# sml2004/CUDA-powered-mesh-handling-and-Iterative-solvers

Measured on NVIDIA B200. Metric: cg_iters_per_s, higher is better.
Workload: dtype f64

## Files before the change

cuda-powered-mesh-handling-and-iterative-solvers_b200/csrc/krylov.cu:

```cuda
#include <cstdlib>

#include "spmv_dev.cuh"

namespace femb {

struct CGState {
  double rs_old, rs_new, pAp, alpha, beta;
  int it, stop, status, iterations;
  unsigned int ticket1, ticket2;
  int fin, fin_status;
};

template <int THREADS>
__device__ __forceinline__ void cg_k1_epilogue_n(double dot, double* __restrict__ partial, CGState* __restrict__ st, double eps, int guards) {
  const double t = block_sum<THREADS>(dot);
  __shared__ bool last;
  if (threadIdx.x == 0) {
    partial[blockIdx.x] = t;
    __threadfence();
    last = atomicAdd(&st->ticket1, 1u) == gridDim.x - 1;
  }
  __syncthreads();
  if (last) {
    __threadfence();
    double a = 0.0;
    for (int k = threadIdx.x; k < (int)gridDim.x; k += THREADS) a += ((volatile double*)partial)[k];
    a = block_sum<THREADS>(a);
    if (threadIdx.x == 0) {
      st->ticket1 = 0;
      st->pAp = a;
      if (guards && (fabs(a) < eps || a < 0.0)) {
        st->stop = 1, st->status = 1, st->iterations = st->it + 1;
      } else {
        const double alpha = st->rs_old / (a + eps);
        st->alpha = alpha;
        if (guards && !isfinite(alpha)) st->stop = 1, st->status = 1, st->iterations = st->it + 1;
      }
    }
  }
}

__device__ __forceinline__ void cg_k1_epilogue(double dot, double* __restrict__ partial, CGState* __restrict__ st, double eps, int guards) {
  cg_k1_epilogue_n<SPMV_THREADS>(dot, partial, st, eps, guards);
}

template <int THREADS>
__device__ __forceinline__ void cg_k1_epilogue3_n(double dot, double e0, double e1, double* __restrict__ partial, CGState* __restrict__ st,
                                                  double eps, int guards, double tol) {
  const double t0 = block_sum<THREADS>(dot), t1 = block_sum<THREADS>(e0), t2 = block_sum<THREADS>(e1);
  const int G = gridDim.x;
  __shared__ bool last;
  if (threadIdx.x == 0) {
    partial[blockIdx.x] = t0, partial[G + blockIdx.x] = t1, partial[2 * G + blockIdx.x] = t2;
    __threadfence();
    last = atomicAdd(&st->ticket1, 1u) == gridDim.x - 1;
  }
  __syncthreads();
  if (last) {
    __threadfence();
    double a = 0.0, b = 0.0, c = 0.0;
    for (int k = threadIdx.x; k < G; k += THREADS)
      a += ((volatile double*)partial)[k], b += ((volatile double*)partial)[G + k], c += ((volatile double*)partial)[2 * G + k];
    a = block_sum<THREADS>(a), b = block_sum<THREADS>(b), c = block_sum<THREADS>(c);
    if (threadIdx.x == 0) {
      st->ticket1 = 0;
      st->pAp = a;
      const double rs = st->rs_old, alpha = rs / (a + eps);
      if (guards && (fabs(a) < eps || a < 0.0 || !isfinite(alpha))) {
        st->stop = 1, st->status = 1, st->iterations = st->it + 1;
      } else {
        double rs_new = rs - 2.0 * alpha * b + alpha * alpha * c;
        if (!(rs_new > 0.0)) rs_new = 0.0;
        const double beta = rs_new / (rs + eps);
        st->alpha = alpha, st->beta = beta, st->rs_new = rs_new;
        st->fin = 0;
        if (guards && !isfinite(beta)) st->fin = 1, st->fin_status = 1;
      }
    }
  }
}

template <int L, bool FUSED>
__global__ void __launch_bounds__(SPMV_THREADS) spmv_kernel(long long n, const int* __restrict__ crow, const int* __restrict__ col,
                                                            const double* __restrict__ val, const double* __restrict__ x,
                                                            double* __restrict__ y, const unsigned char* __restrict__ mask,
                                                            double* __restrict__ partial, CGState* __restrict__ st, double eps, int guards,
                                                            const double* __restrict__ rvec, double tol, const double* __restrict__ wvec) {
  if (st && st->stop) return;
  const bool accumulate = (guards & 2) != 0;
  guards &= 1;
  double e0 = 0.0, e1 = 0.0;
  const int sub = threadIdx.x % L;
  const long long group = (blockIdx.x * (long long)blockDim.x + threadIdx.x) / L;
  const long long ngroups = ((long long)gridDim.x * blockDim.x) / L;
  double dot = 0.0;
  for (long long r0 = 0; r0 < n; r0 += ngroups) {
    const long long r = r0 + group;
    double sum = 0.0;
    if (r < n) {
      const int s = __ldg(crow + r), e = __ldg(crow + r + 1);
      int j = s + sub;
      for (; j + L < e; j += 2 * L) {
        const int c0 = ld_stream(col + j), c1 = ld_stream(col + j + L);
        const double v0 = ld_stream(val + j), v1 = ld_stream(val + j + L);
        sum += v0 * __ldg(x + c0);
        sum += v1 * __ldg(x + c1);
      }
      if (j < e) sum += ld_stream(val + j) * __ldg(x + ld_stream(col + j));
    }
#pragma unroll
    for (int o = L / 2; o > 0; o >>= 1) sum += __shfl_xor_sync(0xffffffffu, sum, o);
    if (r < n && sub == 0) {
      if (accumulate) sum += y[r];
      if (FUSED) {
        if (mask && !mask[r]) sum = 0.0;
        dot += sum * __ldg(x + r);
        if (rvec) {
          const double w = wvec ? wvec[r] : 1.0;
          e0 += sum * (w * rvec[r]), e1 += sum * (sum * w);
        }
      }
      y[r] = sum;
    }
  }
  if (FUSED) {
    if (rvec) cg_k1_epilogue3_n<SPMV_THREADS>(dot, e0, e1, partial, st, eps, guards, tol);
    else cg_k1_epilogue(dot, partial, st, eps, guards);
  }
}

template <int LR, bool FUSED>
__global__ void __launch_bounds__(SPMV_THREADS) spmv_stream_kernel(long long n, const int* __restrict__ crow, const int* __restrict__ col,
                                                                   const double* __restrict__ val, const double* __restrict__ x,
                                                                   double* __restrict__ y, const unsigned char* __restrict__ mask,
                                                                   double* __restrict__ partial, CGState* __restrict__ st, double eps,
                                                                   int guards, const double* __restrict__ rvec, double tol,
                                                                   const double* __restrict__ wvec) {
  if (st && st->stop) return;
  const double dot = spmv_stream_rows<LR, true>(n, crow, col, val, x, y, mask, (guards & 2) != 0, FUSED);
  if (FUSED) cg_k1_epilogue(dot, partial, st, eps, guards & 1);
}

template <int LR, bool FUSED>
__global__ void __launch_bounds__(TMA_THREADS) spmv_tma_kernel(long long n, long long nnz, const int* __restrict__ crow, const int* __restrict__ col,
                                                               const double* __restrict__ val, const double* __restrict__ x,
                                                               double* __restrict__ y, const unsigned char* __restrict__ mask,
                                                               double* __restrict__ partial, CGState* __restrict__ st, double eps, int guards,
                                                               const double* __restrict__ rvec, double tol, long long pin,
                                                               const double* __restrict__ wvec) {
  pdl_launch_dependents();
  double extra[2] = {0.0, 0.0};
  const double dot = spmv_tma_rows<LR, true, TMA_THREADS, TMA_STAGES, TMA_CAP, NoHaloWait, PdlWait>(
      n, nnz, crow, col, val, x, y, mask, (guards & 2) != 0, FUSED, 0x7fffffffffffffffll, NoHaloWait(), rvec, rvec ? extra : nullptr, PdlWait(),
      st ? &st->stop : nullptr, pin, wvec);
  if (st && st->stop) return;
  if (FUSED) {
    if (rvec) cg_k1_epilogue3_n<TMA_THREADS>(dot, extra[0], extra[1], partial, st, eps, guards & 1, tol);
    else cg_k1_epilogue_n<TMA_THREADS>(dot, partial, st, eps, guards & 1);
  }
}

template <bool FUSED>
__global__ void __launch_bounds__(TMA_THREADS) spmv_tma16_kernel(long long n, long long nnz, const int* __restrict__ crow, const int* __restrict__ col,
                                                                 const double* __restrict__ val, const double* __restrict__ x,
                                                                 double* __restrict__ y, const unsigned char* __restrict__ mask,
                                                                 double* __restrict__ partial, CGState* __restrict__ st, double eps, int guards,
                                                                 const double* __restrict__ rvec, double tol, long long pin,
                                                                 const double* __restrict__ wvec, const unsigned short* __restrict__ col16,
                                                                 const unsigned char* __restrict__ tile_ok) {
  pdl_launch_dependents();
  double extra[2] = {0.0, 0.0};
  const double dot = spmv_tma16_rows<TMA16_STAGES, TMA16_CAP>(n, nnz, crow, col, col16, tile_ok, val, x, y, mask, (guards & 2) != 0, FUSED, rvec,
                                                             rvec ? extra : nullptr, st ? &st->stop : nullptr, pin, wvec);
  if (st && st->stop) return;
  if (FUSED) {
    if (rvec) cg_k1_epilogue3_n<TMA_THREADS>(dot, extra[0], extra[1], partial, st, eps, guards & 1, tol);
    else cg_k1_epilogue_n<TMA_THREADS>(dot, partial, st, eps, guards & 1);
  }
}

__global__ void __launch_bounds__(TMA_THREADS) idx16_encode_kernel(long long n, const int* __restrict__ crow, const int* __restrict__ col,
                                                                   unsigned short* __restrict__ col16, unsigned char* __restrict__ tile_ok,
                                                                   int* __restrict__ bad) {
  const long long ntiles = (n + TMA_THREADS - 1) / TMA_THREADS;
  for (long long t = blockIdx.x; t < ntiles; t += gridDim.x) {
    const long long r = t * TMA_THREADS + threadIdx.x;
    bool ok = true;
    if (r < n) {
      const int a = __ldg(crow + r), b = __ldg(crow + r + 1);
      long long prev = r;
      for (int j = a; j < b; ++j) {
        const long long c = __ldg(col + j), d = j == a ? prev - c : c - prev;
        ok = ok && d >= (j == a ? 0 : 1) && d <= 65535;
        col16[j] = (unsigned short)d;
        prev = c;
      }
    }
    ok = __syncthreads_and(ok);
    if (threadIdx.x == 0) {
      tile_ok[t] = ok ? 1 : 0;
      if (!ok) atomicAdd(bad, 1);
    }
  }
}

template <int LR, bool FUSED>
__global__ void __launch_bounds__(TMA_THREADS) spmv_bsr3_tma_kernel(long long nb, long long nnzb, const int* __restrict__ brow,
                                                                    const int* __restrict__ bcol, const double* __restrict__ bval,
                                                                    const double* __restrict__ x, double* __restrict__ y,
                                                                    const unsigned char* __restrict__ mask, double* __restrict__ partial,
                                                                    CGState* __restrict__ st, double eps, int guards,
                                                                    const double* __restrict__ rvec, double tol, const double* __restrict__ wvec) {
  if (st && st->stop) return;
  const double dot = spmv_bsr3_tma_rows<LR, true>(nb, nnzb, brow, bcol, bval, x, y, mask, (guards & 2) != 0, FUSED);
  if (FUSED) cg_k1_epilogue_n<TMA_THREADS>(dot, partial, st, eps, guards & 1);
}

constexpr int BSRV_THREADS = 256;
template <bool FUSED, int U, bool MERGED>
__global__ void __launch_bounds__(BSRV_THREADS) spmv_bsr3_vec_kernel(long long nb, long long nnzb, const int* __restrict__ brow,
                                                                     const int* __restrict__ bcol, const double* __restrict__ bval,
                                                                     const double* __restrict__ x, double* __restrict__ y,
                                                                     const unsigned char* __restrict__ mask, double* __restrict__ partial,
                                                                     CGState* __restrict__ st, double eps, int guards,
                                                                     const double* __restrict__ rvec, double tol, const double* __restrict__ wvec) {
  if (st && st->stop) return;
  const bool accumulate = (guards & 2) != 0;
  guards &= 1;
  double e0 = 0.0, e1 = 0.0;
  const int lane = threadIdx.x & 31;
  const int boff = lane / 9, pos = lane - 9 * boff, cx = pos % 3;
  const bool active = lane < 27;
  const long long gw = (blockIdx.x * (long long)blockDim.x + threadIdx.x) >> 5, nw = ((long long)gridDim.x * blockDim.x) >> 5;
  double dot = 0.0;
  const bool owner = lane == 0 || lane == 3 || lane == 6;
  for (long long r = gw; r < nb; r += nw) {
    const int a = __ldg(brow + r), e = __ldg(brow + r + 1);
    double r_own = 0.0, w_own = 1.0;
    if (MERGED && owner) {
      r_own = rvec[3 * r + lane / 3];
      if (wvec) w_own = wvec[3 * r + lane / 3];
    }
    double acc = 0.0;
    if (active) {
      int b = a + boff;
      for (; b + 3 * (U - 1) < e; b += 3 * U) {
        double v[U], xv[U];
#pragma unroll
        for (int q = 0; q < U; ++q) {
          v[q] = ld_stream(bval + (size_t)(b + 3 * q) * 9 + pos);
          xv[q] = __ldg(x + 3ll * ld_stream(bcol + b + 3 * q) + cx);
        }
#pragma unroll
        for (int q = 0; q < U; ++q) acc += v[q] * xv[q];
      }
      for (; b < e; b += 3) acc += ld_stream(bval + (size_t)b * 9 + pos) * __ldg(x + 3ll * ld_stream(bcol + b) + cx);
    }
    acc += __shfl_down_sync(0xffffffffu, acc, 9) + __shfl_down_sync(0xffffffffu, acc, 18);
    acc += __shfl_down_sync(0xffffffffu, acc, 1) + __shfl_down_sync(0xffffffffu, acc, 2);
    if (lane == 0 || lane == 3 || lane == 6) {
      const long long i = 3 * r + lane / 3;
      double sv = acc;
      if (accumulate) sv += y[i];
      if (FUSED) {
        if (mask && !mask[i]) sv = 0.0;
        dot += sv * __ldg(x + i);
        if (MERGED) e0 += sv * (w_own * r_own), e1 += sv * (sv * w_own);
      }
      y[i] = sv;
    }
  }
  if (FUSED) {
    if (MERGED) cg_k1_epilogue3_n<BSRV_THREADS>(dot, e0, e1, partial, st, eps, guards, tol);
    else cg_k1_epilogue_n<BSRV_THREADS>(dot, partial, st, eps, guards);
  }
}

template <bool TO_BSR>
__global__ void csr_bsr3_permute_kernel(long long nb, const int* __restrict__ brow, const double* __restrict__ in, double* __restrict__ out) {
  const int lane = threadIdx.x & 31;
  const long long w0 = (blockIdx.x * (long long)blockDim.x + threadIdx.x) >> 5, nw = ((long long)gridDim.x * blockDim.x) >> 5;
  for (long long i = w0; i < nb; i += nw) {
    const long long a = brow[i];
    const int len = brow[i + 1] - (int)a, row = 3 * len;
    for (int t = lane; t < 9 * len; t += 32) {
      const int al = t / row, rem = t - al * row, slot = rem / 3, be = rem - 3 * slot;
      const long long ci = 9 * a + t, bi = 9 * (a + slot) + 3 * al + be;
      if (TO_BSR) out[bi] = in[ci];
      else out[ci] = in[bi];
    }
  }
}

__global__ void bsr3_jacobi_kernel(long long nb, const int* __restrict__ brow, const int* __restrict__ bcol, const double* __restrict__ bval,
                                   const unsigned char* __restrict__ mask, double* __restrict__ minv) {
  for (long long r = blockIdx.x * (long long)blockDim.x + threadIdx.x; r < nb; r += (long long)gridDim.x * blockDim.x) {
    int lo = brow[r], hi = brow[r + 1];
    const int end = hi;
    while (lo < hi) {
      const int mid = (lo + hi) >> 1;
      if (bcol[mid] < r) lo = mid + 1;
      else hi = mid;
    }
    const bool found = lo < end && bcol[lo] == r;
    for (int i = 0; i < 3; ++i) {
      const double d = found ? bval[(size_t)lo * 9 + 4 * i] : 0.0;
      minv[3 * r + i] = (d != 0.0 && (!mask || mask[3 * r + i])) ? 1.0 / d : 0.0;
    }
  }
}

constexpr int VEC_THREADS = 256;

__global__ void __launch_bounds__(VEC_THREADS) cg_update_kernel(long long n, double* __restrict__ u, double* __restrict__ r,
                                                                const double* __restrict__ p, const double* __restrict__ Ap,
                                                                const double* __restrict__ minv, double* __restrict__ partial,
                                                                CGState* __restrict__ st, double tol, double eps, int guards, int max_iter) {
  if (st->stop) return;
  const double alpha = st->alpha;
  double dot = 0.0;
  for (long long i = blockIdx.x * (long long)blockDim.x + threadIdx.x; i < n; i += (long long)gridDim.x * blockDim.x) {
    const double pi = p[i], ri = r[i] - alpha * Ap[i];
    u[i] += alpha * pi;
    r[i] = ri;
    dot += minv ? ri * (minv[i] * ri) : ri * ri;
  }
  const double t = block_sum<VEC_THREADS>(dot);
  __shared__ bool last;
  if (threadIdx.x == 0) {
    partial[blockIdx.x] = t;
    __threadfence();
    last = atomicAdd(&st->ticket2, 1u) == gridDim.x - 1;
  }
  __syncthreads();
  if (last) {
    __threadfence();
    double a = 0.0;
    for (int k = threadIdx.x; k < (int)gridDim.x; k += VEC_THREADS) a += ((volatile double*)partial)[k];
    a = block_sum<VEC_THREADS>(a);
    if (threadIdx.x == 0) {
      st->ticket2 = 0;
      st->rs_new = a;
      if (sqrt(a) < tol) {
        st->stop = 1, st->status = 0, st->iterations = st->it + 1;
      } else {
        const double beta = a / (st->rs_old + eps);
        st->beta = beta;
        if (guards && !isfinite(beta)) {
          st->stop = 1, st->status = 1, st->iterations = st->it + 1;
        } else {
          st->rs_old = a;
          st->it += 1;
          if (st->it >= max_iter) st->stop = 2, st->status = 2, st->iterations = max_iter;
        }
      }
    }
  }
}

__global__ void __launch_bounds__(VEC_THREADS) cg_direction_kernel(long long n, const double* __restrict__ r, double* __restrict__ p,
                                                                   const double* __restrict__ minv, const CGState* __restrict__ st) {
  if (st->stop == 1) return;
  const double beta = st->beta;
  for (long long i = blockIdx.x * (long long)blockDim.x + threadIdx.x; i < n; i += (long long)gridDim.x * blockDim.x) {
    const double z = minv ? minv[i] * r[i] : r[i];
    p[i] = z + beta * p[i];
  }
}

__global__ void __launch_bounds__(VEC_THREADS) cg_merged_kernel(long long n, double* __restrict__ u, double* __restrict__ r, double* __restrict__ p,
                                                                const double* __restrict__ Ap, const double* __restrict__ minv,
                                                                double* __restrict__ partial, CGState* __restrict__ st, int max_iter, double tol) {
  pdl_launch_dependents();
  pdl_wait();
  if (st->stop) return;
  const double alpha = st->alpha, beta = st->beta;
  const bool move_p = st->fin == 0;
  double dot = 0.0;
  for (long long i = blockIdx.x * (long long)blockDim.x + threadIdx.x; i < n; i += (long long)gridDim.x * blockDim.x) {
    const double pi = p[i], ri = r[i] - alpha * Ap[i];
    const double zi = minv ? minv[i] * ri : ri;
    u[i] += alpha * pi;
    r[i] = ri;
    dot += ri * zi;
    if (move_p) p[i] = zi + beta * pi;
  }
  const double t = block_sum<VEC_THREADS>(dot);
  __shared__ bool last;
  if (threadIdx.x == 0) {
    partial[blockIdx.x] = t;
    __threadfence();
    last = atomicAdd(&st->ticket2, 1u) == gridDim.x - 1;
  }
  __syncthreads();
  if (last) {
    __threadfence();
    double a = 0.0;
    for (int k = threadIdx.x; k < (int)gridDim.x; k += VEC_THREADS) a += ((volatile double*)partial)[k];
    a = block_sum<VEC_THREADS>(a);
    if (threadIdx.x == 0) {
      st->ticket2 = 0;
      st->rs_new = a;
      if (sqrt(a) < tol) {
        st->stop = 1, st->status = 0, st->iterations = st->it + 1;
      } else if (!move_p) {
        st->stop = 1, st->status = st->fin_status, st->iterations = st->it + 1;
      } else {
        st->rs_old = a;
        st->it += 1;
        if (st->it >= max_iter) st->stop = 2, st->status = 2, st->iterations = max_iter;
      }
    }
  }
}

__global__ void cg_mask_kernel(long long n, double* __restrict__ u, const unsigned char* __restrict__ mask) {
  for (long long i = blockIdx.x * (long long)blockDim.x + threadIdx.x; i < n; i += (long long)gridDim.x * blockDim.x)
    if (!mask[i]) u[i] = 0.0;
}

__global__ void __launch_bounds__(VEC_THREADS) cg_init_kernel(long long n, const double* __restrict__ F, const double* __restrict__ Au,
                                                              const unsigned char* __restrict__ mask, const double* __restrict__ minv,
                                                              double* __restrict__ r, double* __restrict__ p, double* __restrict__ partial) {
  double dot = 0.0;
  for (long long i = blockIdx.x * (long long)blockDim.x + threadIdx.x; i < n; i += (long long)gridDim.x * blockDim.x) {
    double ri = F[i] - Au[i];
    if (mask && !mask[i]) ri = 0.0;
    const double z = minv ? minv[i] * ri : ri;
    r[i] = ri;
    p[i] = z;
    dot += ri * z;
  }
  const double t = block_sum<VEC_THREADS>(dot);
  if (threadIdx.x == 0) partial[blockIdx.x] = t;
}

__global__ void __launch_bounds__(VEC_THREADS) cg_init_finish(int nparts, const double* __restrict__ partial, CGState* __restrict__ st,
                                                              int max_iter) {
  double a = 0.0;
  for (int k = threadIdx.x; k < nparts; k += VEC_THREADS) a += partial[k];
  a = block_sum<VEC_THREADS>(a);
  if (threadIdx.x == 0) {
    CGState s;
    memset(&s, 0, sizeof(s));
    s.rs_old = a;
    s.rs_new = a;
    if (max_iter <= 0) s.stop = 2, s.status = 2;
    *st = s;
  }
}

__global__ void jacobi_kernel(long long n, const int* __restrict__ crow, const int* __restrict__ col, const double* __restrict__ val,
                              const unsigned char* __restrict__ mask, double* __restrict__ minv) {
  for (long long r = blockIdx.x * (long long)blockDim.x + threadIdx.x; r < n; r += (long long)gridDim.x * blockDim.x) {
    double d = 0.0;
    int lo = crow[r], hi = crow[r + 1];
    while (lo < hi) {
      const int mid = (lo + hi) >> 1;
      if (col[mid] < r) lo = mid + 1;
      else hi = mid;
    }
    if (lo < crow[r + 1] && col[lo] == r) d = val[lo];
    minv[r] = (d != 0.0 && (!mask || mask[r])) ? 1.0 / d : 0.0;
  }
}

static int pick_lanes(long long n, long long nnz, int block = 1) {
  static const bool bsr_tma = getenv("FEMB_BSR_TMA") != nullptr;
  static const int bsrv_unroll = getenv("FEMB_BSRV_UNROLL") ? atoi(getenv("FEMB_BSRV_UNROLL")) : 4;
  if (block == 3) return bsr_tma ? 200 + bsr_pick_lr(n / 3, nnz) : (bsrv_unroll == 2 ? 301 : 300);
  const double avg = n > 0 ? (double)nnz / (double)n : 1.0;
  static const bool force_vector = getenv("FEMB_SPMV_VECTOR") != nullptr, force_stream = getenv("FEMB_SPMV_STREAM") != nullptr;
  if (force_vector) return -(avg <= 3 ? 2 : avg <= 6 ? 4 : avg <= 24 ? 8 : avg <= 48 ? 16 : 32);
  static const bool force_tma = getenv("FEMB_SPMV_TMA") != nullptr;
  if (!force_stream && !force_tma && avg >= 64.0) return -32;
  if (!force_stream) return 100 + tma_pick_lr(n, nnz);
  for (int lr = 1; lr <= 32; lr *= 2)
    if ((SPMV_THREADS / lr) * avg * 1.25 <= STREAM_CAP) return lr;
  return 32;
}

static thread_local long long nnz_hint = 0;
static thread_local bool pdl_hint = false;
static thread_local long long pin_hint = 0;
static thread_local const unsigned short* col16_hint = nullptr;
static thread_local const unsigned char* tile_ok_hint = nullptr;

template <bool FUSED>
static void launch_spmv(int lanes, int grid, cudaStream_t s, long long n, const int* crow, const int* col, const double* val, const double* x,
                        double* y, const unsigned char* mask, double* partial, CGState* st, double eps, int guards,
                        const double* rvec = nullptr, double tol = 0.0, const double* wvec = nullptr) {
#define FEMB_SPMV_ARGS n, crow, col, val, x, y, mask, partial, st, eps, guards, rvec, tol, wvec
#define FEMB_TMA(LRV)                                                                                                              \
  {                                                                                                                                \
    cudaFuncSetAttribute(spmv_tma_kernel<LRV, FUSED>, cudaFuncAttributeMaxDynamicSharedMemorySize, (int)TMA_SMEM);                 \
    launch_pdl(spmv_tma_kernel<LRV, FUSED>, grid, TMA_THREADS, TMA_SMEM, s, pdl_hint, n, nnz_hint, crow, col, val, x, y, mask, partial, st, eps, \
               guards, rvec, tol, pin_hint, wvec);                                                                               \
  }
#define FEMB_BSR(LRV)                                                                                                              \
  {                                                                                                                                \
    cudaFuncSetAttribute(spmv_bsr3_tma_kernel<LRV, FUSED>, cudaFuncAttributeMaxDynamicSharedMemorySize, (int)BSR_SMEM);            \
    spmv_bsr3_tma_kernel<LRV, FUSED><<<grid, TMA_THREADS, BSR_SMEM, s>>>(n / 3, nnz_hint, crow, col, val, x, y, mask, partial, st, eps, guards, rvec, tol, wvec); \
  }
  switch (lanes) {
#define FEMB_BSRV(UV)                                                                                                              \
  {                                                                                                                                \
    if (FUSED && rvec)                                                                                                             \
      spmv_bsr3_vec_kernel<FUSED, UV, FUSED><<<grid, BSRV_THREADS, 0, s>>>(n / 3, nnz_hint, crow, col, val, x, y, mask, partial, st, eps, guards, rvec, tol, wvec); \
    else                                                                                                                           \
      spmv_bsr3_vec_kernel<FUSED, UV, false><<<grid, BSRV_THREADS, 0, s>>>(n / 3, nnz_hint, crow, col, val, x, y, mask, partial, st, eps, guards, rvec, tol, wvec); \
  }
    case 300: FEMB_BSRV(4) break;
    case 301: FEMB_BSRV(2) break;
    case 201: FEMB_BSR(1) break;
    case 202: FEMB_BSR(2) break;
    case 204: FEMB_BSR(4) break;
    case 208: FEMB_BSR(8) break;
    case 216: FEMB_BSR(16) break;
    case 232: FEMB_BSR(32) break;
    case 101:
      if (col16_hint) {
        cudaFuncSetAttribute(spmv_tma16_kernel<FUSED>, cudaFuncAttributeMaxDynamicSharedMemorySize, (int)TMA16_SMEM);
        launch_pdl(spmv_tma16_kernel<FUSED>, grid, TMA_THREADS, TMA16_SMEM, s, pdl_hint, n, nnz_hint, crow, col, val, x, y, mask, partial, st,
                   eps, guards, rvec, tol, pin_hint, wvec, col16_hint, tile_ok_hint);
      } else {
        FEMB_TMA(1)
      }
      break;
    case 102: FEMB_TMA(2) break;
    case 104: FEMB_TMA(4) break;
    case 108: FEMB_TMA(8) break;
    case 116: FEMB_TMA(16) break;
    case 132: FEMB_TMA(32) break;
    case 1: spmv_stream_kernel<1, FUSED><<<grid, SPMV_THREADS, 0, s>>>(FEMB_SPMV_ARGS); break;
    case 2: spmv_stream_kernel<2, FUSED><<<grid, SPMV_THREADS, 0, s>>>(FEMB_SPMV_ARGS); break;
    case 4: spmv_stream_kernel<4, FUSED><<<grid, SPMV_THREADS, 0, s>>>(FEMB_SPMV_ARGS); break;
    case 8: spmv_stream_kernel<8, FUSED><<<grid, SPMV_THREADS, 0, s>>>(FEMB_SPMV_ARGS); break;
    case 16: spmv_stream_kernel<16, FUSED><<<grid, SPMV_THREADS, 0, s>>>(FEMB_SPMV_ARGS); break;
    case 32: spmv_stream_kernel<32, FUSED><<<grid, SPMV_THREADS, 0, s>>>(FEMB_SPMV_ARGS); break;
    case -2: spmv_kernel<2, FUSED><<<grid, SPMV_THREADS, 0, s>>>(FEMB_SPMV_ARGS); break;
    case -4: spmv_kernel<4, FUSED><<<grid, SPMV_THREADS, 0, s>>>(FEMB_SPMV_ARGS); break;
    case -8: spmv_kernel<8, FUSED><<<grid, SPMV_THREADS, 0, s>>>(FEMB_SPMV_ARGS); break;
    case -16: spmv_kernel<16, FUSED><<<grid, SPMV_THREADS, 0, s>>>(FEMB_SPMV_ARGS); break;
    default: spmv_kernel<32, FUSED><<<grid, SPMV_THREADS, 0, s>>>(FEMB_SPMV_ARGS); break;
  }
#undef FEMB_TMA
#undef FEMB_BSR
#undef FEMB_BSRV
#undef FEMB_SPMV_ARGS
}

static int spmv_grid(long long n, int lanes, bool merged = false) {
  if (lanes == 300 || lanes == 301) {
    static int fit[2][2] = {{0, 0}, {0, 0}};
    if (!fit[0][0]) {
      cudaOccupancyMaxActiveBlocksPerMultiprocessor(&fit[0][0], spmv_bsr3_vec_kernel<true, 4, false>, BSRV_THREADS, 0);
      cudaOccupancyMaxActiveBlocksPerMultiprocessor(&fit[1][0], spmv_bsr3_vec_kernel<true, 2, false>, BSRV_THREADS, 0);
      cudaOccupancyMaxActiveBlocksPerMultiprocessor(&fit[0][1], spmv_bsr3_vec_kernel<true, 4, true>, BSRV_THREADS, 0);
      cudaOccupancyMaxActiveBlocksPerMultiprocessor(&fit[1][1], spmv_bsr3_vec_kernel<true, 2, true>, BSRV_THREADS, 0);
      for (auto& f : fit)
        for (int& v : f)
          if (v < 1) v = 1;
    }
    const int per_sm = getenv("FEMB_BSRV_CTAS") ? atoi(getenv("FEMB_BSRV_CTAS")) : fit[lanes - 300][merged ? 1 : 0];
    const long long ctas = (n / 3 + BSRV_THREADS / 32 - 1) / (BSRV_THREADS / 32);
    return (int)std::max<long long>(1, std::min<long long>(ctas, (long long)SMS * per_sm));
  }
  if (lanes >= 200) return tma_grid(n / 3, lanes - 200);
  if (lanes >= 100) return tma_grid(n, lanes - 100);
  const long long rows_per_block = SPMV_THREADS / (lanes < 0 ? -lanes : lanes);
  const long long tiles = std::max<long long>(1, (n + rows_per_block - 1) / rows_per_block);
  if (lanes < 0) return (int)std::min<long long>(tiles, (long long)SMS * 8);
  const long long max_ctas = SMS * 32;
  const long long per = (tiles + max_ctas - 1) / max_ctas;
  return (int)((tiles + per - 1) / per);
}

}

using namespace femb;

extern "C" int femb_spmv(int64_t n, int64_t nnz, const int32_t* crow, const int32_t* col, const double* val, const double* x, double* y,
                         femb_stream stream) {
  FEMB_CHECK_ARG(n >= 0, "n >= 0");
  if (n == 0) return FEMB_OK;
  cudaStream_t s = as_stream(stream);
  spmv_apply_env_once();
  const int lanes = pick_lanes(n, nnz);
  nnz_hint = nnz;
  launch_spmv<false>(lanes, spmv_grid(n, lanes), s, n, crow, col, val, x, y, nullptr, nullptr, nullptr, 0.0, 0);
  FEMB_LAUNCH_CHECK();
  return FEMB_OK;
}

extern "C" int femb_csr_jacobi(int64_t n, const int32_t* crow, const int32_t* col, const double* val, const uint8_t* mask, double* minv,
                               femb_stream stream) {
  if (n == 0) return FEMB_OK;
  jacobi_kernel<<<grid_for(n, 256), 256, 0, as_stream(stream)>>>(n, crow, col, val, mask, minv);
  FEMB_LAUNCH_CHECK();
  return FEMB_OK;
}

struct CsrRef {
  long long nnz;
  const int *crow, *col;
  const double* val;
  int block = 1;
};

static int cg_solve_impl(int64_t n, int nmat, const CsrRef* mats, const double* F, const uint8_t* mask, const double* minv, double* u,
                         double* work, double tol, int max_iter, double eps, int check_every, femb_cg_result* result_host,
                         femb_stream stream) {
  FEMB_CHECK_ARG(n > 0 && nmat >= 1 && nmat <= 8 && F && u && work && result_host, "null pointer / n <= 0 / nmat not in 1..8");
  if (check_every < 1) check_every = 16;
  spmv_apply_env_once();
  SolveCtx* ctx = solve_ctx(as_stream(stream));
  if (!ctx) return FEMB_ERR_CUDA;
  cudaStream_t s = ctx->stream;
  const int guards = minv ? 0 : 1;
  if (minv) eps = 0.0;
  double *r = work, *p = work + n, *Ap = work + 2 * n;
  int lanes[8], g1[8], gmax = 1;
  for (int m = 0; m < nmat; ++m) lanes[m] = pick_lanes(n, mats[m].nnz, mats[m].block);
  static const bool classic_env = getenv("FEMB_CG_CLASSIC") != nullptr;
  const int ll = lanes[nmat - 1];
  static const bool bsr_merged = getenv("FEMB_BSR_MERGED") != nullptr;
  const bool merged = !classic_env && ((ll >= 300 && bsr_merged) || (ll >= 100 && ll < 200) || ll < 0);
  static const bool idx32_env = getenv("FEMB_SPMV_IDX32") != nullptr;
  bool use16 = !idx32_env && merged && nmat == 1 && lanes[0] == 101 && max_iter >= 16;
  const long long ntiles16 = (n + TMA_THREADS - 1) / TMA_THREADS;
  const size_t flags_off = 256, col16_off = flags_off + (((size_t)ntiles16 + 255) & ~(size_t)255);
  if (use16) {
    const size_t need16 = col16_off + 2 * (((size_t)mats[0].nnz + 7) & ~(size_t)7);
    if (ctx->idx16_bytes < need16) {
      if (ctx->graph_exec) cudaGraphExecDestroy(ctx->graph_exec), ctx->graph_exec = nullptr, ctx->graph_key_bytes = 0;
      FEMB_CUDA(cudaStreamSynchronize(s));
      if (ctx->idx16) cudaFree(ctx->idx16);
      ctx->idx16 = nullptr, ctx->idx16_bytes = 0;
      if (cudaMalloc(&ctx->idx16, need16) == cudaSuccess) ctx->idx16_bytes = need16;
      else ctx->idx16 = nullptr, use16 = false, cudaGetLastError();
    }
  }
  if (use16) {
    unsigned char* base16 = static_cast<unsigned char*>(ctx->idx16);
    static_assert(2 * sizeof(CGState) + sizeof(int) <= 512 && 512 + sizeof(int) <= SOLVE_PINNED_BYTES, "pinned status buffer");
    int* bad_host = reinterpret_cast<int*>(static_cast<unsigned char*>(ctx->pinned) + 512);
    FEMB_CUDA(cudaMemsetAsync(base16, 0, sizeof(int), s));
    idx16_encode_kernel<<<(int)std::min<long long>(ntiles16, (long long)SMS * 16), TMA_THREADS, 0, s>>>(
        n, mats[0].crow, mats[0].col, reinterpret_cast<unsigned short*>(base16 + col16_off), base16 + flags_off, reinterpret_cast<int*>(base16));
    FEMB_LAUNCH_CHECK();
    FEMB_CUDA(cudaMemcpyAsync(bad_host, base16, sizeof(int), cudaMemcpyDeviceToHost, s));
    FEMB_CUDA(cudaStreamSynchronize(s));
    use16 = (long long)*bad_host * 100 <= ntiles16;
  }
  const unsigned short* col16 = use16 ? reinterpret_cast<const unsigned short*>(static_cast<unsigned char*>(ctx->idx16) + col16_off) : nullptr;
  const unsigned char* tile_ok = use16 ? static_cast<unsigned char*>(ctx->idx16) + flags_off : nullptr;
  for (int m = 0; m < nmat; ++m) {
    g1[m] = spmv_grid(n, lanes[m], merged && m == nmat - 1);
    if (use16) g1[m] = tma16_grid(n);
    gmax = std::max(gmax, g1[m]);
  }
  const int g2 = grid_for(n, VEC_THREADS, 8);
  static const int vec_waves = getenv("FEMB_VEC_WAVES") ? atoi(getenv("FEMB_VEC_WAVES")) : 8;
  const int g2v = grid_for(n, VEC_THREADS, vec_waves);
  const size_t need = 256 + sizeof(double) * (size_t)std::max(3 * gmax, g2);
  if (ctx->dev_scratch_bytes < need) {
    if (ctx->graph_exec) cudaGraphExecDestroy(ctx->graph_exec), ctx->graph_exec = nullptr, ctx->graph_key_bytes = 0;
    FEMB_CUDA(cudaStreamSynchronize(s));
    if (ctx->dev_scratch) cudaFree(ctx->dev_scratch);
    ctx->dev_scratch = nullptr, ctx->dev_scratch_bytes = 0;
    FEMB_CUDA(cudaMalloc(&ctx->dev_scratch, need + need / 2));
    ctx->dev_scratch_bytes = need + need / 2;
  }
  static_assert(sizeof(CGState) <= 256, "state slot");
  CGState* st = static_cast<CGState*>(ctx->dev_scratch);
  double* partial = reinterpret_cast<double*>(static_cast<unsigned char*>(ctx->dev_scratch) + 256);
  if (mask) cg_mask_kernel<<<g2, VEC_THREADS, 0, s>>>(n, u, mask);
  col16_hint = col16, tile_ok_hint = tile_ok;
  for (int m = 0; m < nmat; ++m)
    nnz_hint = mats[m].nnz, launch_spmv<false>(lanes[m], g1[m], s, n, mats[m].crow, mats[m].col, mats[m].val, u, Ap, nullptr, nullptr, nullptr, 0.0, m ? 2 : 0);
  col16_hint = nullptr, tile_ok_hint = nullptr;
  cg_init_kernel<<<g2, VEC_THREADS, 0, s>>>(n, F, Ap, mask, minv, r, p, partial);
  cg_init_finish<<<1, VEC_THREADS, 0, s>>>(g2, partial, st, max_iter);
  FEMB_LAUNCH_CHECK();
  struct GraphKey {
    long long n;
    int nmat, check_every, max_iter, guards, merged, pdl, lanes[8], g1[8], g2, g2v;
    long long nnz[8];
    const void *crow[8], *col[8], *val[8];
    int block[8];
    const void *mask, *minv, *u, *work, *st, *partial;
    double tol, eps;
    long long pin;
    const void* col16;
  } key;
  memset(&key, 0, sizeof(key));
  static_assert(sizeof(GraphKey) <= sizeof(ctx->graph_key), "graph key buffer");
  key.n = n, key.nmat = nmat, key.check_every = check_every, key.max_iter = max_iter, key.guards = guards, key.merged = merged ? 1 : 0;
  key.pdl = pdl_mode(), key.g2 = g2, key.g2v = g2v, key.mask = mask, key.minv = minv, key.u = u, key.work = work, key.st = st, key.partial = partial;
  key.tol = tol, key.eps = eps, key.pin = spmv_pin_entries(mats[nmat - 1].nnz), key.col16 = col16;
  for (int m = 0; m < nmat; ++m) {
    key.lanes[m] = lanes[m], key.g1[m] = g1[m];
    key.nnz[m] = mats[m].nnz, key.crow[m] = mats[m].crow, key.col[m] = mats[m].col, key.val[m] = mats[m].val, key.block[m] = mats[m].block;
  }
  static const bool no_cache = getenv("FEMB_NO_GRAPH_CACHE") != nullptr;
  cudaGraph_t graph = nullptr;
  cudaGraphExec_t exec = nullptr;
  if (!no_cache && ctx->graph_exec && ctx->graph_key_bytes == sizeof(key) && memcmp(ctx->graph_key, &key, sizeof(key)) == 0) exec = ctx->graph_exec;
  if (!exec) {
  FEMB_CUDA(cudaStreamBeginCapture(s, cudaStreamCaptureModeThreadLocal));
  for (int k = 0; k < check_every; ++k) {
    for (int m = 0; m + 1 < nmat; ++m)
      nnz_hint = mats[m].nnz, launch_spmv<false>(lanes[m], g1[m], s, n, mats[m].crow, mats[m].col, mats[m].val, p, Ap, nullptr, nullptr, st, 0.0, m ? 2 : 0);
    const int last = nmat - 1;
    nnz_hint = mats[last].nnz;
    if (merged) {
      const bool pdl = pdl_enabled() && nmat == 1 && lanes[last] >= 100 && lanes[last] < 200;
      pdl_hint = pdl && k > 0 && (pdl_mode() & 2);
      pin_hint = pdl ? spmv_pin_entries(mats[last].nnz) : 0;
      col16_hint = col16, tile_ok_hint = tile_ok;
      launch_spmv<true>(lanes[last], g1[last], s, n, mats[last].crow, mats[last].col, mats[last].val, p, Ap, mask, partial, st, eps,
                        guards | (last ? 2 : 0), r, tol, minv);
      pdl_hint = false, pin_hint = 0, col16_hint = nullptr, tile_ok_hint = nullptr;
      launch_pdl(cg_merged_kernel, g2v, VEC_THREADS, 0, s, pdl && (pdl_mode() & 1), n, u, r, p, Ap, minv, partial, st, max_iter, tol);
    } else {
      launch_spmv<true>(lanes[last], g1[last], s, n, mats[last].crow, mats[last].col, mats[last].val, p, Ap, mask, partial, st, eps,
                        guards | (last ? 2 : 0));
      cg_update_kernel<<<g2, VEC_THREADS, 0, s>>>(n, u, r, p, Ap, minv, partial, st, tol, eps, guards, max_iter);
      cg_direction_kernel<<<g2, VEC_THREADS, 0, s>>>(n, r, p, minv, st);
    }
  }
  cudaError_t ce = cudaStreamEndCapture(s, &graph);
  if (ce != cudaSuccess) {
    set_error(std::string("cudaStreamEndCapture: ") + cudaGetErrorString(ce));
    return FEMB_ERR_CUDA;
  }
  FEMB_CUDA(cudaGraphInstantiate(&exec, graph, 0));
  cudaGraphDestroy(graph);
  FEMB_CUDA(cudaGraphUpload(exec, s));
  if (ctx->graph_exec) cudaGraphExecDestroy(ctx->graph_exec);
  ctx->graph_exec = exec, ctx->graph_key_bytes = sizeof(key);
  memcpy(ctx->graph_key, &key, sizeof(key));
  }
  static_assert(2 * sizeof(CGState) <= SOLVE_PINNED_BYTES, "pinned status buffer");
  CGState* hst = static_cast<CGState*>(ctx->pinned);
  cudaEvent_t* ev = ctx->poll_ev;
  cudaEvent_t* tev = ctx->time_ev;
  int rc = FEMB_OK;
  const int launches = (max_iter + check_every - 1) / check_every;
  hst[0].stop = hst[1].stop = 0;
  bool stopped = false;
  cudaEventRecord(tev[0], s);
  for (int l = 0; l < launches && !stopped; ++l) {
    if (cudaGraphLaunch(exec, s) != cudaSuccess || cudaMemcpyAsync(&hst[l & 1], st, sizeof(CGState), cudaMemcpyDeviceToHost, s) != cudaSuccess ||
        cudaEventRecord(ev[l & 1], s) != cudaSuccess) {
      set_error(std::string("CG graph launch: ") + cudaGetErrorString(cudaGetLastError()));
      rc = FEMB_ERR_CUDA;
      break;
    }
    if (l >= 1) {
      cudaEventSynchronize(ev[(l - 1) & 1]);
      stopped = hst[(l - 1) & 1].stop != 0;
    }
  }
  cudaEventRecord(tev[1], s);
  CGState* fin = &hst[0];
  if (rc == FEMB_OK) {
    if (cudaMemcpyAsync(fin, st, sizeof(CGState), cudaMemcpyDeviceToHost, s) != cudaSuccess || cudaStreamSynchronize(s) != cudaSuccess) {
      set_error(std::string("CG final state: ") + cudaGetErrorString(cudaGetLastError()));
      rc = FEMB_ERR_CUDA;
    }
  }
  float ms = 0.f;
  if (rc == FEMB_OK) cudaEventElapsedTime(&ms, tev[0], tev[1]);
  if (rc != FEMB_OK) {
    cudaGraphExecDestroy(ctx->graph_exec);
    ctx->graph_exec = nullptr, ctx->graph_key_bytes = 0;
    return rc;
  }
  result_host->iterations = fin->stop ? fin->iterations : max_iter;
  result_host->status = fin->stop ? fin->status : 2;
  result_host->rs = fin->rs_new;
  result_host->loop_ms = ms;
  result_host->index_bytes = use16 ? 2 : 4;
  return FEMB_OK;
}

extern "C" int femb_cg_solve(int64_t n, int64_t nnz, const int32_t* crow, const int32_t* col, const double* val, const double* F,
                             const uint8_t* mask, const double* minv, double* u, double* work, double tol, int max_iter, double eps,
                             int check_every, femb_cg_result* result_host, femb_stream stream) {
  FEMB_CHECK_ARG(crow && col && val, "null CSR pointer");
  const CsrRef m{nnz, crow, col, val, 1};
  return cg_solve_impl(n, 1, &m, F, mask, minv, u, work, tol, max_iter, eps, check_every, result_host, stream);
}

extern "C" int femb_spmv_bsr3(int64_t nb, int64_t nnzb, const int32_t* brow, const int32_t* bcol, const double* bval, const double* x,
                              double* y, femb_stream stream) {
  FEMB_CHECK_ARG(nb >= 0 && nnzb >= 0, "nb >= 0, nnzb >= 0");
  if (nb == 0) return FEMB_OK;
  cudaStream_t s = as_stream(stream);
  const int lanes = pick_lanes(3 * nb, nnzb, 3);
  nnz_hint = nnzb;
  launch_spmv<false>(lanes, spmv_grid(3 * nb, lanes), s, 3 * nb, brow, bcol, bval, x, y, nullptr, nullptr, nullptr, 0.0, 0);
  FEMB_LAUNCH_CHECK();
  return FEMB_OK;
}

extern "C" int femb_cg_solve_bsr3(int64_t nb, int64_t nnzb, const int32_t* brow, const int32_t* bcol, const double* bval, const double* F,
                                  const uint8_t* mask, const double* minv, double* u, double* work, double tol, int max_iter, double eps,
                                  int check_every, femb_cg_result* result_host, femb_stream stream) {
  FEMB_CHECK_ARG(brow && bcol && bval, "null BSR pointer");
  const CsrRef m{nnzb, brow, bcol, bval, 3};
  return cg_solve_impl(3 * nb, 1, &m, F, mask, minv, u, work, tol, max_iter, eps, check_every, result_host, stream);
}

extern "C" int femb_csr_bsr3_convert(int to_bsr, int64_t nb, const int32_t* brow, const double* in, double* out, femb_stream stream) {
  FEMB_CHECK_ARG(nb >= 0 && brow && in && out && in != out, "nb >= 0, non-null distinct buffers");
  if (nb == 0) return FEMB_OK;
  const int grid = grid_for(nb * 32, 256, 32);
  if (to_bsr) csr_bsr3_permute_kernel<true><<<grid, 256, 0, as_stream(stream)>>>(nb, brow, in, out);
  else csr_bsr3_permute_kernel<false><<<grid, 256, 0, as_stream(stream)>>>(nb, brow, in, out);
  FEMB_LAUNCH_CHECK();
  return FEMB_OK;
}

extern "C" int femb_bsr3_jacobi(int64_t nb, const int32_t* brow, const int32_t* bcol, const double* bval, const uint8_t* mask, double* minv,
                                femb_stream stream) {
  if (nb == 0) return FEMB_OK;
  bsr3_jacobi_kernel<<<grid_for(nb, 256), 256, 0, as_stream(stream)>>>(nb, brow, bcol, bval, mask, minv);
  FEMB_LAUNCH_CHECK();
  return FEMB_OK;
}

extern "C" int femb_cg_solve_multi(int64_t n, int nmat, const int64_t* nnz_host, const int32_t* const* crow_host,
                                   const int32_t* const* col_host, const double* const* val_host, const double* F, const uint8_t* mask,
                                   const double* minv, double* u, double* work, double tol, int max_iter, double eps, int check_every,
                                   femb_cg_result* result_host, femb_stream stream) {
  FEMB_CHECK_ARG(nmat >= 1 && nmat <= 8 && nnz_host && crow_host && col_host && val_host, "nmat in 1..8, non-null arrays");
  CsrRef m[8];
  for (int k = 0; k < nmat; ++k) m[k] = CsrRef{nnz_host[k], crow_host[k], col_host[k], val_host[k], 1};
  return cg_solve_impl(n, nmat, m, F, mask, minv, u, work, tol, max_iter, eps, check_every, result_host, stream);
}

namespace femb {

__global__ void __launch_bounds__(VEC_THREADS) cg_dot_kernel(long long n, const double* __restrict__ p, const double* __restrict__ Ap,
                                                             double* __restrict__ partial, CGState* __restrict__ st) {
  if (st->stop) return;
  double dot = 0.0;
  for (long long i = blockIdx.x * (long long)blockDim.x + threadIdx.x; i < n; i += (long long)gridDim.x * blockDim.x) dot += p[i] * Ap[i];
  cg_k1_epilogue_n<VEC_THREADS>(dot, partial, st, 0.0, 0);
}

}

extern "C" int femb_cg_solve_operator(int64_t n, femb_apply_fn apply, void* ctx, const double* R, double* u, double* work, double tol,
                                      int max_iter, int check_every, femb_cg_result* result_host, femb_stream stream) {
  FEMB_CHECK_ARG(n > 0 && apply && R && u && work && result_host, "null pointer / n <= 0");
  if (check_every < 1) check_every = 8;
  cudaStream_t s = as_stream(stream);
  double *r = work, *p = work + n, *Ap = work + 2 * n;
  const int g2 = grid_for(n, VEC_THREADS, 8);
  Scratch scr(s);
  double* partial;
  CGState* st;
  FEMB_CUDA(scr.alloc(&partial, (size_t)g2));
  FEMB_CUDA(scr.alloc(&st, 1));
  cudaEvent_t t0, t1;
  FEMB_CUDA(cudaEventCreate(&t0));
  FEMB_CUDA(cudaEventCreate(&t1));
  int rc = FEMB_OK;
  CGState h;
  memset(&h, 0, sizeof(h));
  auto fail = [&](const char* what) {
    set_error(what);
    rc = FEMB_ERR_ARG;
  };
  if (apply(ctx, u, Ap, stream) != 0) fail("femb_cg_solve_operator: the operator callback failed");
  if (rc == FEMB_OK) {
    cg_init_kernel<<<g2, VEC_THREADS, 0, s>>>(n, R, Ap, nullptr, nullptr, r, p, partial);
    cg_init_finish<<<1, VEC_THREADS, 0, s>>>(g2, partial, st, max_iter);
    cudaEventRecord(t0, s);
    for (int it = 0; it < max_iter && rc == FEMB_OK; ++it) {
      if (apply(ctx, p, Ap, stream) != 0) {
        fail("femb_cg_solve_operator: the operator callback failed");
        break;
      }
      cg_dot_kernel<<<g2, VEC_THREADS, 0, s>>>(n, p, Ap, partial, st);
      cg_update_kernel<<<g2, VEC_THREADS, 0, s>>>(n, u, r, p, Ap, nullptr, partial, st, tol, 0.0, 0, max_iter);
      cg_direction_kernel<<<g2, VEC_THREADS, 0, s>>>(n, r, p, nullptr, st);
      if ((it + 1) % check_every == 0 || it + 1 == max_iter) {
        if (cudaMemcpyAsync(&h, st, sizeof(CGState), cudaMemcpyDeviceToHost, s) != cudaSuccess || cudaStreamSynchronize(s) != cudaSuccess) {
          set_error(std::string("femb_cg_solve_operator: ") + cudaGetErrorString(cudaGetLastError()));
          rc = FEMB_ERR_CUDA;
          break;
        }
        if (h.stop) break;
      }
    }
    cudaEventRecord(t1, s);
  }
  if (rc == FEMB_OK) {
    if (cudaMemcpyAsync(&h, st, sizeof(CGState), cudaMemcpyDeviceToHost, s) != cudaSuccess || cudaStreamSynchronize(s) != cudaSuccess) {
      set_error(std::string("femb_cg_solve_operator: ") + cudaGetErrorString(cudaGetLastError()));
      rc = FEMB_ERR_CUDA;
    }
  }
  float ms = 0.f;
  if (rc == FEMB_OK) cudaEventElapsedTime(&ms, t0, t1);
  cudaEventDestroy(t0);
  cudaEventDestroy(t1);
  if (rc != FEMB_OK) {
    cudaStreamSynchronize(s);
    return rc;
  }
  result_host->iterations = h.stop ? h.iterations : max_iter;
  result_host->status = h.stop ? h.status : 2;
  result_host->rs = h.rs_new;
  result_host->loop_ms = ms;
  result_host->index_bytes = 0;
  return FEMB_OK;
}
```

cuda-powered-mesh-handling-and-iterative-solvers_b200/csrc/spmv_dev.cuh:

```cuda
#pragma once
#include <cstdlib>

#include "common.cuh"

namespace femb {

constexpr int SPMV_THREADS = 256;
constexpr int STREAM_CAP = 5632;

__device__ __forceinline__ double ld_stream(const double* p) {
  double v;
  asm volatile("ld.global.nc.L1::no_allocate.f64 %0, [%1];" : "=d"(v) : "l"(p));
  return v;
}
__device__ __forceinline__ int ld_stream(const int* p) {
  int v;
  asm volatile("ld.global.nc.L1::no_allocate.s32 %0, [%1];" : "=r"(v) : "l"(p));
  return v;
}
template <bool NC>
__device__ __forceinline__ double ld_x(const double* p) {
  if (NC) return __ldg(p);
  return *p;
}

struct NoHaloWait {
  __device__ __forceinline__ void operator()() const {}
};

template <int LR, bool NC, typename Wait = NoHaloWait>
__device__ __forceinline__ double spmv_stream_rows(long long n, const int* __restrict__ crow, const int* __restrict__ col,
                                                   const double* __restrict__ val, const double* __restrict__ x, double* __restrict__ y,
                                                   const unsigned char* __restrict__ mask, bool accumulate, bool fused,
                                                   long long halo_row = 0x7fffffffffffffffll, Wait wait = Wait()) {
  constexpr int R = SPMV_THREADS / LR;
  __shared__ double prod[STREAM_CAP];
  __shared__ int rp[R + 1];
  const int tid = threadIdx.x, sub = tid % LR, lr = tid / LR;
  double dot = 0.0;
  bool waited = false;
  for (long long r0 = (long long)blockIdx.x * R; r0 < n; r0 += (long long)gridDim.x * R) {
    const int nr = (int)min((long long)R, n - r0);
    if (!waited && r0 + nr > halo_row) {
      wait();
      waited = true;
    }
    double x_own = 0.0, y_prev = 0.0;
    bool keep = true;
    if (lr < nr && sub == 0) {
      if (fused) {
        x_own = ld_x<NC>(x + r0 + lr);
        if (mask) keep = mask[r0 + lr] != 0;
      }
      if (accumulate) y_prev = y[r0 + lr];
    }
    for (int t = tid; t <= nr; t += SPMV_THREADS) rp[t] = __ldg(crow + r0 + t);
    __syncthreads();
    const int s = rp[0], e = rp[nr];
    const bool fits = (e - s) <= STREAM_CAP;
    if (fits) {
      int j = s + tid;
      for (; j + 3 * SPMV_THREADS < e; j += 4 * SPMV_THREADS) {
        int c[4];
        double v[4];
#pragma unroll
        for (int q = 0; q < 4; ++q) c[q] = ld_stream(col + j + q * SPMV_THREADS), v[q] = ld_stream(val + j + q * SPMV_THREADS);
#pragma unroll
        for (int q = 0; q < 4; ++q) prod[j - s + q * SPMV_THREADS] = v[q] * ld_x<NC>(x + c[q]);
      }
      for (; j < e; j += SPMV_THREADS) prod[j - s] = ld_stream(val + j) * ld_x<NC>(x + ld_stream(col + j));
    }
    __syncthreads();
    double sum = 0.0;
    if (lr < nr) {
      const int a = rp[lr], b = rp[lr + 1];
      if (fits) {
        for (int j = a - s + sub; j < b - s; j += LR) sum += prod[j];
      } else {
        for (int j = a + sub; j < b; j += LR) sum += ld_stream(val + j) * ld_x<NC>(x + ld_stream(col + j));
      }
    }
#pragma unroll
    for (int o = LR / 2; o > 0; o >>= 1) sum += __shfl_xor_sync(0xffffffffu, sum, o);
    if (lr < nr && sub == 0) {
      const long long r = r0 + lr;
      if (accumulate) sum += y_prev;
      if (fused) {
        if (!keep) sum = 0.0;
        dot += sum * x_own;
      }
      y[r] = sum;
    }
    __syncthreads();
  }
  return dot;
}

__device__ __forceinline__ unsigned smem_u32(const void* p) { return static_cast<unsigned>(__cvta_generic_to_shared(p)); }
__device__ __forceinline__ void mbar_init(unsigned long long* bar, unsigned count) {
  asm volatile("mbarrier.init.shared::cta.b64 [%0], %1;" ::"r"(smem_u32(bar)), "r"(count));
}
__device__ __forceinline__ void mbar_expect_tx(unsigned long long* bar, unsigned bytes) {
  asm volatile("mbarrier.arrive.expect_tx.shared::cta.b64 _, [%0], %1;" ::"r"(smem_u32(bar)), "r"(bytes) : "memory");
}
__device__ __forceinline__ void mbar_wait(unsigned long long* bar, unsigned parity) {
  asm volatile(
      "{\n\t.reg .pred p;\n\t"
      "WAIT_LOOP:\n\t"
      "mbarrier.try_wait.parity.shared::cta.b64 p, [%0], %1;\n\t"
      "@p bra WAIT_DONE;\n\t"
      "bra WAIT_LOOP;\n\t"
      "WAIT_DONE:\n\t}" ::"r"(smem_u32(bar)),
      "r"(parity)
      : "memory");
}
__device__ __forceinline__ void bulk_g2s(void* dst, const void* src, unsigned bytes, unsigned long long* bar) {
  asm volatile("cp.async.bulk.shared::cluster.global.mbarrier::complete_tx::bytes [%0], [%1], %2, [%3];" ::"r"(smem_u32(dst)), "l"(src),
               "r"(bytes), "r"(smem_u32(bar))
               : "memory");
}

__device__ __forceinline__ unsigned long long l2_evict_first_policy() {
  unsigned long long pol;
  asm volatile("createpolicy.fractional.L2::evict_first.b64 %0, 1.0;" : "=l"(pol));
  return pol;
}
__device__ __forceinline__ void bulk_g2s_hint(void* dst, const void* src, unsigned bytes, unsigned long long* bar, unsigned long long pol) {
  asm volatile("cp.async.bulk.shared::cluster.global.mbarrier::complete_tx::bytes.L2::cache_hint [%0], [%1], %2, [%3], %4;" ::"r"(smem_u32(dst)),
               "l"(src), "r"(bytes), "r"(smem_u32(bar)), "l"(pol)
               : "memory");
}
__device__ __forceinline__ unsigned long long l2_evict_last_policy() {
  unsigned long long pol;
  asm volatile("createpolicy.fractional.L2::evict_last.b64 %0, 1.0;" : "=l"(pol));
  return pol;
}
static __device__ int g_spmv_l2_hint = 1;
static inline void spmv_apply_env_once() {
  static thread_local int done_for = -1;
  int dev = 0;
  if (cudaGetDevice(&dev) != cudaSuccess || dev == done_for) return;
  done_for = dev;
  if (const char* e = getenv("FEMB_SPMV_L2HINT")) {
    const int v = atoi(e);
    cudaMemcpyToSymbol(g_spmv_l2_hint, &v, sizeof(int));
  }
}
inline long long spmv_pin_entries(long long nnz) {
  static const double env_mb = getenv("FEMB_SPMV_PIN_MB") ? atof(getenv("FEMB_SPMV_PIN_MB")) : -1.0;
  const double bytes = 12.0 * (double)nnz;
  double pin_mb = env_mb;
  if (pin_mb < 0.0) pin_mb = 0.0;
  return (long long)std::min(bytes, pin_mb * 1e6) / 12;
}

__device__ __forceinline__ void pdl_launch_dependents() { asm volatile("griddepcontrol.launch_dependents;" ::: "memory"); }
__device__ __forceinline__ void pdl_wait() { asm volatile("griddepcontrol.wait;" ::: "memory"); }
struct PdlWait {
  __device__ __forceinline__ void operator()() const { pdl_wait(); }
};
struct NoDep {
  __device__ __forceinline__ void operator()() const {}
};

template <typename... KArgs, typename... Args>
inline cudaError_t launch_pdl(void (*kern)(KArgs...), int grid, int block, size_t smem, cudaStream_t s, bool pdl, Args... args) {
  cudaLaunchConfig_t cfg = {};
  cfg.gridDim = dim3((unsigned)grid), cfg.blockDim = dim3((unsigned)block), cfg.dynamicSmemBytes = smem, cfg.stream = s;
  cudaLaunchAttribute at[1];
  at[0].id = cudaLaunchAttributeProgrammaticStreamSerialization;
  at[0].val.programmaticStreamSerializationAllowed = 1;
  cfg.attrs = at, cfg.numAttrs = pdl ? 1 : 0;
  return cudaLaunchKernelEx(&cfg, kern, static_cast<KArgs>(args)...);
}
inline int pdl_mode() {
  static const int m = getenv("FEMB_NO_PDL") ? 0 : (getenv("FEMB_PDL_MODE") ? atoi(getenv("FEMB_PDL_MODE")) : 2);
  return m;
}
inline bool pdl_enabled() { return pdl_mode() != 0; }

constexpr int TMA_THREADS = 128, TMA_STAGES = 2, TMA_CAP = 2304, TMA_CTAS_PER_SM = 4;
constexpr size_t TMA_SMEM = (size_t)TMA_STAGES * TMA_CAP * 12;

template <int LR, bool NC, int THREADS = TMA_THREADS, int STAGES = TMA_STAGES, int CAP = TMA_CAP, typename Wait = NoHaloWait,
          typename Dep = NoDep>
__device__ __forceinline__ double spmv_tma_rows(long long n, long long nnz, const int* __restrict__ crow, const int* __restrict__ col,
                                                const double* __restrict__ val, const double* __restrict__ x, double* __restrict__ y,
                                                const unsigned char* __restrict__ mask, bool accumulate, bool fused,
                                                long long halo_row = 0x7fffffffffffffffll, Wait wait = Wait(),
                                                const double* __restrict__ rvec = nullptr, double* extra = nullptr, Dep dep = Dep(),
                                                const int* stop = nullptr, long long pin = 0, const double* __restrict__ wvec = nullptr) {
  constexpr int R = THREADS / LR;
  extern __shared__ __align__(128) unsigned char tma_smem[];
  double* vbuf = reinterpret_cast<double*>(tma_smem);
  int* cbuf = reinterpret_cast<int*>(tma_smem + sizeof(double) * STAGES * CAP);
  __shared__ unsigned long long full[STAGES];
  __shared__ int base[STAGES];
  const int tid = threadIdx.x, sub = tid % LR, lr = tid / LR;
  const long long ntiles = (n + R - 1) / R;
  const bool use_hint = g_spmv_l2_hint != 0;
  const unsigned long long pol = l2_evict_first_policy(), pol_keep = l2_evict_last_policy();
  if (tid == 0) {
    for (int s = 0; s < STAGES; ++s) mbar_init(&full[s], 1);
    asm volatile("fence.mbarrier_init.release.cluster;" ::: "memory");
  }
  __syncthreads();
  auto bounds = [&](long long k, int& a, int& b) {
    const long long t = blockIdx.x + k * gridDim.x;
    a = b = 0;
    if (t < ntiles) a = __ldg(crow + t * R), b = __ldg(crow + min(n, t * R + R));
  };
  auto stage_tile = [&](long long k, int a, int b) {
    if (blockIdx.x + k * gridDim.x >= ntiles) return;
    const int s = (int)(k % STAGES);
    const int a0 = a & ~3, cnt = (b - a0 + 3) & ~3;
    if (cnt > CAP || (long long)a0 + cnt > nnz || cnt == 0) {
      base[s] = -1;
      return;
    }
    base[s] = a0;
    asm volatile("fence.proxy.async.shared::cta;" ::: "memory");
    mbar_expect_tx(&full[s], (unsigned)cnt * 12u);
    if (use_hint) {
      const unsigned long long pl = (long long)a0 + cnt <= pin ? pol_keep : pol;
      bulk_g2s_hint(vbuf + (size_t)s * CAP, val + a0, (unsigned)cnt * 8u, &full[s], pl);
      bulk_g2s_hint(cbuf + (size_t)s * CAP, col + a0, (unsigned)cnt * 4u, &full[s], pl);
    } else {
      bulk_g2s(vbuf + (size_t)s * CAP, val + a0, (unsigned)cnt * 8u, &full[s]);
      bulk_g2s(cbuf + (size_t)s * CAP, col + a0, (unsigned)cnt * 4u, &full[s]);
    }
  };
  int na = 0, nb = 0;
  if (tid == 0) {
    for (int k = 0; k < STAGES - 1; ++k) {
      bounds(k, na, nb);
      stage_tile(k, na, nb);
    }
    bounds(STAGES - 1, na, nb);
  }
  double dot = 0.0;
  unsigned phase_bits = 0;
  bool waited = false;
  dep();
  if (stop) {
    __shared__ int stop_sh;
    if (tid == 0) stop_sh = *(volatile const int*)stop;
    __syncthreads();
    if (stop_sh) {
      for (int k = 0; k < STAGES - 1; ++k)
        if (blockIdx.x + (long long)k * gridDim.x < ntiles && base[k % STAGES] >= 0) mbar_wait(&full[k % STAGES], 0u);
      return 0.0;
    }
  }
  for (long long k = 0;; ++k) {
    const long long t = blockIdx.x + k * gridDim.x;
    if (t >= ntiles) break;
    const int s = (int)(k % STAGES);
    if (!waited && min(n, t * R + R) > halo_row) {
      wait();
      waited = true;
    }
    if (tid == 0) {
      stage_tile(k + STAGES - 1, na, nb);
      bounds(k + STAGES, na, nb);
    }
    const long long r = t * R + lr;
    int ra = 0, rb = 0;
    double x_own = 0.0, y_prev = 0.0, r_own = 0.0, w_own = 1.0;
    bool keep = true;
    if (r < n) {
      ra = __ldg(crow + r), rb = __ldg(crow + r + 1);
      if (sub == 0) {
        if (fused) {
          x_own = ld_x<NC>(x + r);
          if (mask) keep = mask[r] != 0;
          if (rvec) r_own = rvec[r];
          if (wvec) w_own = wvec[r];
        }
        if (accumulate) y_prev = y[r];
      }
    }
    __syncthreads();
    const int a0 = base[s];
    double sum = 0.0;
    if (a0 >= 0) {
      mbar_wait(&full[s], (phase_bits >> s) & 1u);
      phase_bits ^= 1u << s;
      const double* vs = vbuf + (size_t)s * CAP - a0;
      const int* cs = cbuf + (size_t)s * CAP - a0;
      int j = ra + sub;
      for (; j + 7 * LR < rb; j += 8 * LR) {
        double xv[8];
#pragma unroll
        for (int q = 0; q < 8; ++q) xv[q] = ld_x<NC>(x + cs[j + q * LR]);
#pragma unroll
        for (int q = 0; q < 8; ++q) sum += vs[j + q * LR] * xv[q];
      }
      {
        double xv[7];
#pragma unroll
        for (int q = 0; q < 7; ++q) xv[q] = (j + q * LR < rb) ? ld_x<NC>(x + cs[j + q * LR]) : 0.0;
#pragma unroll
        for (int q = 0; q < 7; ++q)
          if (j + q * LR < rb) sum += vs[j + q * LR] * xv[q];
      }
    } else {
      for (int j = ra + sub; j < rb; j += LR) sum += ld_stream(val + j) * ld_x<NC>(x + ld_stream(col + j));
    }
#pragma unroll
    for (int o = LR / 2; o > 0; o >>= 1) sum += __shfl_xor_sync(0xffffffffu, sum, o);
    if (r < n && sub == 0) {
      if (accumulate) sum += y_prev;
      if (fused) {
        if (!keep) sum = 0.0;
        dot += sum * x_own;
        if (extra) extra[0] += sum * (w_own * r_own), extra[1] += sum * (sum * w_own);
      }
      y[r] = sum;
    }
    __syncthreads();
  }
  return dot;
}

inline int tma_pick_lr(long long n, long long nnz) {
  const double avg = n > 0 ? (double)nnz / (double)n : 1.0;
  for (int lr = 1; lr <= 32; lr *= 2)
    if ((TMA_THREADS / lr) * avg * 1.15 <= TMA_CAP) return lr;
  return 32;
}
inline int tma_grid(long long n, int lr) {
  const long long tiles = (n + TMA_THREADS / lr - 1) / (TMA_THREADS / lr);
  return (int)std::max<long long>(1, std::min<long long>(tiles, (long long)SMS * TMA_CTAS_PER_SM));
}

#ifndef FEMB_TMA16_STAGES
#define FEMB_TMA16_STAGES 2
#endif
#ifndef FEMB_TMA16_CAP
#define FEMB_TMA16_CAP 2176
#endif
#ifndef FEMB_TMA16_CTAS
#define FEMB_TMA16_CTAS 5
#endif
constexpr int TMA16_STAGES = FEMB_TMA16_STAGES, TMA16_CAP = FEMB_TMA16_CAP, TMA16_CTAS_PER_SM = FEMB_TMA16_CTAS;
constexpr size_t TMA16_SMEM = (size_t)TMA16_STAGES * TMA16_CAP * 10;
inline int tma16_grid(long long n) {
  const long long tiles = (n + TMA_THREADS - 1) / TMA_THREADS;
  return (int)std::max<long long>(1, std::min<long long>(tiles, (long long)SMS * TMA16_CTAS_PER_SM));
}

template <int STAGES, int CAP>
__device__ __forceinline__ double spmv_tma16_rows(long long n, long long nnz, const int* __restrict__ crow, const int* __restrict__ col,
                                                  const unsigned short* __restrict__ col16, const unsigned char* __restrict__ tile_ok,
                                                  const double* __restrict__ val, const double* __restrict__ x, double* __restrict__ y,
                                                  const unsigned char* __restrict__ mask, bool accumulate, bool fused,
                                                  const double* __restrict__ rvec, double* extra, const int* stop, long long pin,
                                                  const double* __restrict__ wvec) {
  static_assert(CAP % 8 == 0, "16-byte aligned stages");
  constexpr int R = TMA_THREADS;
  extern __shared__ __align__(128) unsigned char tma_smem[];
  double* vbuf = reinterpret_cast<double*>(tma_smem);
  unsigned short* dbuf = reinterpret_cast<unsigned short*>(tma_smem + sizeof(double) * STAGES * CAP);
  __shared__ unsigned long long full[STAGES];
  __shared__ int base[STAGES];
  const int tid = threadIdx.x;
  const long long ntiles = (n + R - 1) / R;
  const bool use_hint = g_spmv_l2_hint != 0;
  const unsigned long long pol = l2_evict_first_policy(), pol_keep = l2_evict_last_policy();
  if (tid == 0) {
    for (int s = 0; s < STAGES; ++s) mbar_init(&full[s], 1);
    asm volatile("fence.mbarrier_init.release.cluster;" ::: "memory");
  }
  __syncthreads();
  auto bounds = [&](long long k, int& a, int& b, int& ok) {
    const long long t = blockIdx.x + k * gridDim.x;
    a = b = ok = 0;
    if (t < ntiles) a = __ldg(crow + t * R), b = __ldg(crow + min(n, t * R + R)), ok = __ldg(tile_ok + t);
  };
  auto stage_tile = [&](long long k, int a, int b, int ok) {
    if (blockIdx.x + k * gridDim.x >= ntiles) return;
    const int s = (int)(k % STAGES);
    const int a0 = a & ~7, cnt = (b - a0 + 7) & ~7, cntv = (b - a0 + 1) & ~1;
    if (!ok || cnt > CAP || (long long)a0 + cntv > nnz || b == a) {
      base[s] = -1;
      return;
    }
    base[s] = a0;
    asm volatile("fence.proxy.async.shared::cta;" ::: "memory");
    mbar_expect_tx(&full[s], (unsigned)cntv * 8u + (unsigned)cnt * 2u);
    if (use_hint) {
      const unsigned long long pl = (long long)a0 + cntv <= pin ? pol_keep : pol;
      bulk_g2s_hint(vbuf + (size_t)s * CAP, val + a0, (unsigned)cntv * 8u, &full[s], pl);
      bulk_g2s_hint(dbuf + (size_t)s * CAP, col16 + a0, (unsigned)cnt * 2u, &full[s], pl);
    } else {
      bulk_g2s(vbuf + (size_t)s * CAP, val + a0, (unsigned)cntv * 8u, &full[s]);
      bulk_g2s(dbuf + (size_t)s * CAP, col16 + a0, (unsigned)cnt * 2u, &full[s]);
    }
  };
  int na = 0, nb = 0, nok = 0;
  if (tid == 0) {
    for (int k = 0; k < STAGES - 1; ++k) {
      bounds(k, na, nb, nok);
      stage_tile(k, na, nb, nok);
    }
    bounds(STAGES - 1, na, nb, nok);
  }
  double dot = 0.0;
  unsigned phase_bits = 0;
  pdl_wait();
  if (stop) {
    __shared__ int stop_sh;
    if (tid == 0) stop_sh = *(volatile const int*)stop;
    __syncthreads();
    if (stop_sh) {
      for (int k = 0; k < STAGES - 1; ++k)
        if (blockIdx.x + (long long)k * gridDim.x < ntiles && base[k % STAGES] >= 0) mbar_wait(&full[k % STAGES], 0u);
      return 0.0;
    }
  }
  for (long long k = 0;; ++k) {
    const long long t = blockIdx.x + k * gridDim.x;
    if (t >= ntiles) break;
    const int s = (int)(k % STAGES);
    if (tid == 0) {
      stage_tile(k + STAGES - 1, na, nb, nok);
      bounds(k + STAGES, na, nb, nok);
    }
    const long long r = t * R + tid;
    int ra = 0, rb = 0;
    double x_own = 0.0, y_prev = 0.0, r_own = 0.0, w_own = 1.0;
    bool keep = true;
    if (r < n) {
      ra = __ldg(crow + r), rb = __ldg(crow + r + 1);
      if (fused) {
        x_own = __ldg(x + r);
        if (mask) keep = mask[r] != 0;
        if (rvec) r_own = rvec[r];
        if (wvec) w_own = wvec[r];
      }
      if (accumulate) y_prev = y[r];
    }
    __syncthreads();
    const int a0 = base[s];
    double sum = 0.0;
    if (a0 >= 0) {
      mbar_wait(&full[s], (phase_bits >> s) & 1u);
      phase_bits ^= 1u << s;
      const double* vs = vbuf + (size_t)s * CAP - a0;
      const unsigned short* ds = dbuf + (size_t)s * CAP - a0;
      int c = ra < rb ? (int)r - 2 * (int)ds[ra] : 0;
      int j = ra;
      for (; j + 7 < rb; j += 8) {
        double xv[8];
#pragma unroll
        for (int q = 0; q < 8; ++q) c += ds[j + q], xv[q] = __ldg(x + c);
#pragma unroll
        for (int q = 0; q < 8; ++q) sum += vs[j + q] * xv[q];
      }
      {
        double xv[7];
#pragma unroll
        for (int q = 0; q < 7; ++q) {
          if (j + q < rb) c += ds[j + q];
          xv[q] = (j + q < rb) ? __ldg(x + c) : 0.0;
        }
#pragma unroll
        for (int q = 0; q < 7; ++q)
          if (j + q < rb) sum += vs[j + q] * xv[q];
      }
    } else {
      for (int j = ra; j < rb; ++j) sum += ld_stream(val + j) * __ldg(x + ld_stream(col + j));
    }
    if (r < n) {
      if (accumulate) sum += y_prev;
      if (fused) {
        if (!keep) sum = 0.0;
        dot += sum * x_own;
        if (extra) extra[0] += sum * (w_own * r_own), extra[1] += sum * (sum * w_own);
      }
      y[r] = sum;
    }
    __syncthreads();
  }
  return dot;
}

constexpr int BSR_CAP = 352;
constexpr size_t BSR_SMEM = (size_t)TMA_STAGES * BSR_CAP * 76;

template <int LR, bool NC, int THREADS = TMA_THREADS, int STAGES = TMA_STAGES, int CAP = BSR_CAP>
__device__ __forceinline__ double spmv_bsr3_tma_rows(long long nb, long long nnzb, const int* __restrict__ brow, const int* __restrict__ bcol,
                                                     const double* __restrict__ bval, const double* __restrict__ x, double* __restrict__ y,
                                                     const unsigned char* __restrict__ mask, bool accumulate, bool fused) {
  constexpr int R = THREADS / LR;
  extern __shared__ __align__(128) unsigned char tma_smem[];
  double* vbuf = reinterpret_cast<double*>(tma_smem);
  int* cbuf = reinterpret_cast<int*>(tma_smem + sizeof(double) * 9 * STAGES * CAP);
  __shared__ unsigned long long full[STAGES];
  __shared__ int base[STAGES];
  const int tid = threadIdx.x, sub = tid % LR, lr = tid / LR;
  const long long ntiles = (nb + R - 1) / R;
  if (tid == 0) {
    for (int s = 0; s < STAGES; ++s) mbar_init(&full[s], 1);
    asm volatile("fence.mbarrier_init.release.cluster;" ::: "memory");
  }
  __syncthreads();
  auto bounds = [&](long long k, int& a, int& b) {
    const long long t = blockIdx.x + k * gridDim.x;
    a = b = 0;
    if (t < ntiles) a = __ldg(brow + t * R), b = __ldg(brow + min(nb, t * R + R));
  };
  auto stage_tile = [&](long long k, int a, int b) {
    if (blockIdx.x + k * gridDim.x >= ntiles) return;
    const int s = (int)(k % STAGES);
    const int a0 = a & ~3, cnt = (b - a0 + 3) & ~3;
    if (cnt > CAP || (long long)a0 + cnt > nnzb || cnt == 0) {
      base[s] = -1;
      return;
    }
    base[s] = a0;
    asm volatile("fence.proxy.async.shared::cta;" ::: "memory");
    mbar_expect_tx(&full[s], (unsigned)cnt * 76u);
    bulk_g2s(vbuf + (size_t)s * CAP * 9, bval + (size_t)a0 * 9, (unsigned)cnt * 72u, &full[s]);
    bulk_g2s(cbuf + (size_t)s * CAP, bcol + a0, (unsigned)cnt * 4u, &full[s]);
  };
  int na = 0, nbnd = 0;
  if (tid == 0) {
    for (int k = 0; k < STAGES - 1; ++k) {
      bounds(k, na, nbnd);
      stage_tile(k, na, nbnd);
    }
    bounds(STAGES - 1, na, nbnd);
  }
  double dot = 0.0;
  unsigned phase_bits = 0;
  for (long long k = 0;; ++k) {
    const long long t = blockIdx.x + k * gridDim.x;
    if (t >= ntiles) break;
    const int s = (int)(k % STAGES);
    if (tid == 0) {
      stage_tile(k + STAGES - 1, na, nbnd);
      bounds(k + STAGES, na, nbnd);
    }
    const long long r = t * R + lr;
    int ra = 0, rb = 0;
    double xo[3] = {0, 0, 0}, yp[3] = {0, 0, 0};
    bool keep[3] = {true, true, true};
    if (r < nb) {
      ra = __ldg(brow + r), rb = __ldg(brow + r + 1);
      if (sub == 0) {
#pragma unroll
        for (int i = 0; i < 3; ++i) {
          if (fused) {
            xo[i] = ld_x<NC>(x + 3 * r + i);
            if (mask) keep[i] = mask[3 * r + i] != 0;
          }
          if (accumulate) yp[i] = y[3 * r + i];
        }
      }
    }
    __syncthreads();
    const int a0 = base[s];
    double s0 = 0.0, s1 = 0.0, s2 = 0.0;
    if (a0 >= 0) {
      mbar_wait(&full[s], (phase_bits >> s) & 1u);
      phase_bits ^= 1u << s;
      const double* vs = vbuf + (size_t)s * CAP * 9 - (size_t)a0 * 9;
      const int* cs = cbuf + (size_t)s * CAP - a0;
      int j = ra + sub;
      for (; j + 3 * LR < rb; j += 4 * LR) {
        double xv[4][3];
#pragma unroll
        for (int q = 0; q < 4; ++q) {
          const double* xp = x + 3ll * cs[j + q * LR];
          xv[q][0] = ld_x<NC>(xp), xv[q][1] = ld_x<NC>(xp + 1), xv[q][2] = ld_x<NC>(xp + 2);
        }
#pragma unroll
        for (int q = 0; q < 4; ++q) {
          const double* b = vs + (size_t)(j + q * LR) * 9;
          s0 += b[0] * xv[q][0] + b[1] * xv[q][1] + b[2] * xv[q][2];
          s1 += b[3] * xv[q][0] + b[4] * xv[q][1] + b[5] * xv[q][2];
          s2 += b[6] * xv[q][0] + b[7] * xv[q][1] + b[8] * xv[q][2];
        }
      }
      {
        double xv[3][3];
#pragma unroll
        for (int q = 0; q < 3; ++q) {
          const bool in = j + q * LR < rb;
          const double* xp = x + 3ll * (in ? cs[j + q * LR] : 0);
          xv[q][0] = in ? ld_x<NC>(xp) : 0.0, xv[q][1] = in ? ld_x<NC>(xp + 1) : 0.0, xv[q][2] = in ? ld_x<NC>(xp + 2) : 0.0;
        }
#pragma unroll
        for (int q = 0; q < 3; ++q)
          if (j + q * LR < rb) {
            const double* b = vs + (size_t)(j + q * LR) * 9;
            s0 += b[0] * xv[q][0] + b[1] * xv[q][1] + b[2] * xv[q][2];
            s1 += b[3] * xv[q][0] + b[4] * xv[q][1] + b[5] * xv[q][2];
            s2 += b[6] * xv[q][0] + b[7] * xv[q][1] + b[8] * xv[q][2];
          }
      }
    } else {
      for (int j = ra + sub; j < rb; j += LR) {
        const double* b = bval + (size_t)j * 9;
        const double* xp = x + 3ll * ld_stream(bcol + j);
        const double x0 = ld_x<NC>(xp), x1 = ld_x<NC>(xp + 1), x2 = ld_x<NC>(xp + 2);
        s0 += ld_stream(b) * x0 + ld_stream(b + 1) * x1 + ld_stream(b + 2) * x2;
        s1 += ld_stream(b + 3) * x0 + ld_stream(b + 4) * x1 + ld_stream(b + 5) * x2;
        s2 += ld_stream(b + 6) * x0 + ld_stream(b + 7) * x1 + ld_stream(b + 8) * x2;
      }
    }
#pragma unroll
    for (int o = LR / 2; o > 0; o >>= 1) {
      s0 += __shfl_xor_sync(0xffffffffu, s0, o);
      s1 += __shfl_xor_sync(0xffffffffu, s1, o);
      s2 += __shfl_xor_sync(0xffffffffu, s2, o);
    }
    if (r < nb && sub == 0) {
      double sv[3] = {s0, s1, s2};
#pragma unroll
      for (int i = 0; i < 3; ++i) {
        if (accumulate) sv[i] += yp[i];
        if (fused) {
          if (!keep[i]) sv[i] = 0.0;
          dot += sv[i] * xo[i];
        }
        y[3 * r + i] = sv[i];
      }
    }
    __syncthreads();
  }
  return dot;
}

inline int bsr_pick_lr(long long nb, long long nnzb) {
  const double avg = nb > 0 ? (double)nnzb / (double)nb : 1.0;
  for (int lr = 1; lr <= 32; lr *= 2)
    if ((TMA_THREADS / lr) * avg * 1.15 <= BSR_CAP) return lr;
  return 32;
}

}
```

cuda-powered-mesh-handling-and-iterative-solvers_b200/femb200/_lib.py:

```python
from __future__ import annotations

import ctypes as C
import os

_HERE = os.path.dirname(os.path.abspath(__file__))
LIB_PATH = os.path.join(os.path.dirname(_HERE), "libfemb200.so")

c_i32, c_i64, c_f64, c_vp = C.c_int, C.c_int64, C.c_double, C.c_void_p


class CGResult(C.Structure):
    _fields_ = [("iterations", C.c_int32), ("status", C.c_int32), ("rs", C.c_double), ("loop_ms", C.c_double),
                ("index_bytes", C.c_int32)]


APPLY_FN = C.CFUNCTYPE(C.c_int, c_vp, c_vp, c_vp, c_vp)

SIGNATURES = {
    "femb_version": [],
    "femb_elem_volumes": [c_i32, c_vp, c_i32, c_vp, c_i32, c_i64, c_i32, c_vp, c_vp],
    "femb_c3d4": [c_i32, c_vp, c_i32, c_vp, c_i32, c_i64, c_f64, c_f64, c_vp, c_vp, c_vp],
    "femb_solid": [c_i32, c_i32, c_vp, c_i32, c_vp, c_i32, c_i64, C.POINTER(c_f64), c_i32, c_f64, c_f64, c_vp, c_vp],
    "femb_default_points": [c_i32, C.POINTER(c_f64)],
    "femb_mass_points": [c_i32, C.POINTER(c_f64)],
    "femb_solid_stress": [c_i32, c_vp, c_i32, c_vp, c_i32, c_i64, c_vp, C.POINTER(c_f64), c_i32, c_f64, c_f64, c_i32, c_vp, c_vp, c_vp],
    "femb_shape_tables": [c_i32, C.POINTER(c_f64), c_i32, C.POINTER(c_f64), C.POINTER(c_f64)],
    "femb_stress_helper": [c_i32, c_vp, c_i32, c_i64, c_vp, c_vp],
    "femb_node_average": [c_vp, c_vp, c_i32, c_vp, c_vp],
    "femb_shell": [c_i32, c_i32, c_vp, c_i32, c_vp, c_i32, c_i64, C.POINTER(c_f64), c_i32, C.POINTER(c_f64), c_vp, c_vp],
    "femb_shell_ex": [c_i32, c_i32, c_vp, c_i32, c_vp, c_i32, c_i64, C.POINTER(c_f64), c_i32, C.POINTER(c_f64), c_vp, c_vp, c_vp],
    "femb_shell_normal": [c_vp, c_i32, c_vp, c_i32, c_i64, c_i32, c_vp, c_vp],
    "femb_shell_rotate_operator": [c_vp, c_vp, c_i32, c_i64, c_i32, c_vp, c_vp],
    "femb_shell_local_coordinates": [c_vp, c_i32, c_vp, c_i32, c_i64, c_i32, c_vp, c_vp, c_vp],
    "femb_shell_local_displacement": [c_vp, c_i32, c_i64, c_i32, c_vp, c_vp, c_i32, c_vp, c_vp],
    "femb_shell_postprocess": [c_vp, c_i32, c_i64, c_i32, c_f64, c_f64, c_vp, c_vp],
    "femb_face_forces": [c_vp, c_vp, c_i32, c_i64, c_i32, c_vp, c_vp],
    "femb_shared_face_forces_sum": [c_vp, c_i64, c_vp, c_i32, c_i32, c_vp, c_vp],
    "femb_wedge_face_normals": [c_vp, c_i32, c_vp, c_i32, c_i64, c_i32, c_vp, c_vp],
    "femb_shell_extrude": [c_vp, c_vp, c_vp, c_i32, c_i64, c_f64, c_f64, c_vp, c_vp],
    "femb_extrude_connectivity": [c_vp, c_i32, c_i64, c_i32, c_i64, c_vp, c_vp],
    "femb_to_c3d4": [c_i32, c_vp, c_i32, c_i64, c_vp, c_vp],
    "femb_p2_create": [c_vp, c_i32, c_i64, c_i64, c_vp, C.POINTER(c_vp), C.POINTER(c_i64)],
    "femb_p2_fill": [c_vp, c_vp, c_i32, c_vp, c_i32, c_i32, c_vp, c_vp, c_vp, c_vp],
    "femb_p2_destroy": [c_vp],
    "femb_entities_create": [c_i32, c_vp, c_i32, c_i64, c_i32, c_vp, C.POINTER(c_vp), C.POINTER(c_i64), C.POINTER(c_i64)],
    "femb_entities_surface": [c_vp, c_vp, c_vp, c_vp],
    "femb_entities_shared": [c_vp, c_vp, c_vp],
    "femb_entities_destroy": [c_vp],
    "femb_surface_normals": [c_vp, c_i32, c_vp, c_vp, c_i64, c_i32, c_i32, c_vp, c_vp],
    "femb_face_normals_area": [c_i32, c_vp, c_i32, c_vp, c_i32, c_i64, c_i32, c_vp, c_vp],
    "femb_csr_plan_create": [c_vp, c_i32, c_i64, c_i32, c_i64, c_vp, C.POINTER(c_vp), C.POINTER(c_i64)],
    "femb_csr_plan_pattern": [c_vp, c_i32, c_vp, c_vp, c_vp],
    "femb_csr_assemble": [c_vp, c_i32, c_vp, c_vp, c_vp],
    "femb_csr_assemble_c3d4": [c_vp, c_i32, c_vp, c_f64, c_f64, c_vp, c_vp, c_vp],
    "femb_csr_plan_destroy": [c_vp],
    "femb_spmv": [c_i64, c_i64, c_vp, c_vp, c_vp, c_vp, c_vp, c_vp],
    "femb_ebe_apply": [c_vp, c_i32, c_vp, c_vp, c_vp, c_i32, c_vp, c_vp],
    "femb_cg_solve": [c_i64, c_i64, c_vp, c_vp, c_vp, c_vp, c_vp, c_vp, c_vp, c_vp, c_f64, c_i32, c_f64, c_i32,
                      C.POINTER(CGResult), c_vp],
    "femb_cg_solve_bsr3": [c_i64, c_i64, c_vp, c_vp, c_vp, c_vp, c_vp, c_vp, c_vp, c_vp, c_f64, c_i32, c_f64, c_i32,
                           C.POINTER(CGResult), c_vp],
    "femb_spmv_bsr3": [c_i64, c_i64, c_vp, c_vp, c_vp, c_vp, c_vp, c_vp],
    "femb_csr_bsr3_convert": [c_i32, c_i64, c_vp, c_vp, c_vp, c_vp],
    "femb_bsr3_jacobi": [c_i64, c_vp, c_vp, c_vp, c_vp, c_vp, c_vp],
    "femb_cg_solve_multi": [c_i64, c_i32, C.POINTER(c_i64), C.POINTER(c_vp), C.POINTER(c_vp), C.POINTER(c_vp), c_vp, c_vp, c_vp, c_vp,
                            c_vp, c_f64, c_i32, c_f64, c_i32, C.POINTER(CGResult), c_vp],
    "femb_cg_solve_operator": [c_i64, APPLY_FN, c_vp, c_vp, c_vp, c_vp, c_f64, c_i32, c_i32, C.POINTER(CGResult), c_vp],
    "femb_vtk_open": [C.c_char_p, C.POINTER(c_vp), C.POINTER(c_i64), C.POINTER(c_i64), C.POINTER(c_i64), C.POINTER(C.c_int32)],
    "femb_vtk_read": [c_vp, c_vp, c_vp, c_vp],
    "femb_vtk_close": [c_vp],
    "femb_ebe_diag": [c_vp, c_i32, c_vp, c_i32, c_i32, c_vp, c_vp],
    "femb_mv_gram": [c_i64, c_i32, c_vp, c_i64, c_i32, c_vp, c_i64, c_vp, C.POINTER(c_f64), c_vp],
    "femb_mv_update": [c_i64, c_i32, c_vp, c_i64, c_i32, C.POINTER(c_f64), c_f64, c_vp, c_i64, c_vp],
    "femb_mv_scale_mask": [c_i64, c_i32, c_vp, c_i64, c_vp, c_vp, c_vp],
    "femb_spmm_bsr3": [c_i64, c_i64, c_vp, c_vp, c_vp, c_vp, c_vp, c_i32, c_vp, c_i64, c_vp, c_vp, c_i64, c_vp],
    "femb_mb_gram": [c_i64, c_i32, c_vp, c_i64, c_i32, c_vp, c_i64, c_vp, c_vp],
    "femb_mb_combine": [c_i64, c_i32, c_vp, c_i64, c_i32, C.POINTER(c_f64), c_f64, c_vp, c_i64, c_vp],
    "femb_lobpcg_residual": [c_i64, c_i32, c_vp, c_i64, c_vp, c_vp, c_i64, C.POINTER(c_f64), c_vp, c_i32, c_vp, c_vp, c_i64, c_vp, c_vp],
    "femb_csr_jacobi": [c_i64, c_vp, c_vp, c_vp, c_vp, c_vp, c_vp],
    "femb_graph_from_pairs": [c_vp, c_i64, c_i32, c_i64, c_vp, c_vp, c_vp],
    "femb_subdomain_forces": [c_vp, c_i32, c_i64, c_i32, c_vp, c_i64, c_vp, c_vp, c_vp, c_vp, c_vp],
    "femb_graph_bfs": [c_vp, c_vp, c_i64, c_vp, c_i32, c_vp, c_vp, C.POINTER(c_i32), c_vp],
    "femb_dist_header_bytes": [],
    "femb_dist_alloc": [c_i64, C.POINTER(c_vp), c_vp],
    "femb_dist_open": [c_vp, C.POINTER(c_vp)],
    "femb_dist_close": [c_vp],
    "femb_dist_free": [c_vp],
    "femb_dist_reset": [c_vp, c_vp],
    "femb_dist_cg_solve": [c_i32, c_i32, c_i64, c_i64, c_i64, c_vp, c_vp, c_vp, c_vp, c_vp, c_vp, c_vp, c_vp, C.POINTER(c_vp), c_i32,
                           C.POINTER(C.c_int32), C.POINTER(C.c_int32), c_vp, C.POINTER(c_i64), c_vp, c_vp, c_vp, c_f64, c_i32, c_f64, c_i32,
                           c_i32, C.POINTER(CGResult), c_vp],
}
_RESTYPES = {"femb_last_error": C.c_char_p}


class FembError(RuntimeError):
    pass


def _load():
    if not os.path.exists(LIB_PATH):
        raise ImportError(
            f"{LIB_PATH} is missing: build it with `python -c 'import __graft_entry__ as g; g.build()'` "
            "(or `make -C <package>/csrc`).  There is no CPU fallback.")
    lib = C.CDLL(LIB_PATH)
    lib.femb_last_error.restype = C.c_char_p
    lib.femb_last_error.argtypes = []
    for name, args in SIGNATURES.items():
        fn = getattr(lib, name)
        fn.argtypes = args
        fn.restype = C.c_int
    return lib


lib = _load()


def check(rc: int, what: str = ""):
    if rc != 0:
        msg = lib.femb_last_error().decode("utf-8", "replace")
        raise FembError(f"{what} failed (status {rc}): {msg}")
```

cuda-powered-mesh-handling-and-iterative-solvers_b200/femb200/ops.py:

```python
from __future__ import annotations

import collections
import ctypes as C
import os
import weakref

import torch

from . import _lib
from ._lib import CGResult, check, lib

C3D4, C3D6, C3D8, C3D10, C3D15, C3D20, S3, S4 = 4, 6, 8, 10, 15, 20, 103, 104
ENT_TET_FACES, ENT_HEX_FACES, ENT_WEDGE_QUADS, ENT_WEDGE_TRIS, ENT_TRI_EDGES, ENT_QUAD_EDGES = range(6)
_ENT = {ENT_TET_FACES: (4, 3), ENT_HEX_FACES: (6, 4), ENT_WEDGE_QUADS: (3, 4), ENT_WEDGE_TRIS: (2, 3), ENT_TRI_EDGES: (3, 2),
        ENT_QUAD_EDGES: (4, 2)}


def cuda_device(device) -> torch.device:
    d = torch.device(device)
    if d.type != "cuda":
        raise RuntimeError(f"femb200 runs on CUDA devices only (got device={device!r}); there is no CPU fallback")
    if not torch.cuda.is_available():
        raise RuntimeError("femb200 needs a CUDA device (sm_100a); none is visible")
    return d


def _stream(dev) -> int:
    return torch.cuda.current_stream(dev).cuda_stream


def real(t, dev, dtype) -> torch.Tensor:
    if dtype not in (torch.float32, torch.float64):
        raise TypeError(f"dtype must be float32 or float64, got {dtype}")
    return torch.as_tensor(t).to(device=dev, dtype=dtype).contiguous()


def index(t, dev) -> torch.Tensor:
    t = torch.as_tensor(t).to(device=dev)
    if t.dtype not in (torch.int32, torch.int64):
        t = t.to(torch.int64)
    return t.contiguous()


def _fp(t):
    return t.element_size()


def _p(t):
    return C.c_void_p(t.data_ptr()) if t is not None else C.c_void_p(0)


def _host_doubles(values):
    arr = (C.c_double * len(values))(*[float(v) for v in values])
    return arr


def default_points(kind) -> list:
    buf = (C.c_double * (64 * 4))()
    n = lib.femb_default_points(kind, buf)
    if n < 0:
        check(1, "femb_default_points")
    return [[buf[4 * q + k] for k in range(4)] for q in range(n)]


def mass_points(kind) -> list:
    buf = (C.c_double * (64 * 4))()
    n = lib.femb_mass_points(kind, buf)
    if n < 0:
        check(1, "femb_mass_points")
    return [[buf[4 * q + k] for k in range(4)] for q in range(n)]



def _out_buffer(out, shape, dev, dtype):
    if out is None:
        return torch.empty(shape, device=dev, dtype=dtype)
    if tuple(out.shape) != tuple(shape) or out.dtype != dtype or out.device != torch.device(dev) or not out.is_contiguous():
        raise ValueError(f"out= must be a contiguous {dtype} tensor of shape {tuple(shape)} on {dev}")
    return out


def c3d4(what, coords, elements, E=0.0, nu=0.0, device="cuda:0", dtype=torch.float32, out=None):
    dev = cuda_device(device)
    x, conn = real(coords, dev, dtype), index(elements, dev)
    M = conn.shape[0]
    shape = {0: (M, 4, 3), 1: (M, 6, 12), 2: (M, 12, 12), 3: (M, 4, 4), 4: (M, 12, 12), 5: (M,)}[what]
    out = _out_buffer(out, shape, dev, dtype)
    flag = torch.zeros(1, device=dev, dtype=torch.int32)
    with torch.cuda.device(dev):
        check(lib.femb_c3d4(what, _p(x), _fp(x), _p(conn), _fp(conn), M, float(E), float(nu), _p(out), _p(flag), _stream(dev)), "femb_c3d4")
    if what in (0, 1, 2, 3) and M and int(flag.item()):
        raise ValueError("Singular matrix encountered while computing B matrix.")
    return out


def volumes(kind, coords, elements, device="cuda:0", dtype=torch.float32):
    dev = cuda_device(device)
    x, conn = real(coords, dev, dtype), index(elements, dev)
    M = conn.shape[0]
    out = torch.empty((M,), device=dev, dtype=dtype)
    with torch.cuda.device(dev):
        check(lib.femb_elem_volumes(kind, _p(x), _fp(x), _p(conn), _fp(conn), M, conn.shape[1], _p(out), _stream(dev)), "femb_elem_volumes")
    return out


_NEN = {C3D4: 4, C3D6: 6, C3D8: 8, C3D10: 10, C3D15: 15, C3D20: 20, S3: 3, S4: 4}


def solid(kind, what, coords, elements, points, E=0.0, nu=0.0, device="cuda:0", dtype=torch.float32, out=None):
    dev = cuda_device(device)
    x, conn = real(coords, dev, dtype), index(elements, dev)
    nen = _NEN[kind]
    if conn.shape[1] != nen:
        conn = conn[:, :nen].contiguous()
    M, nd, nq = conn.shape[0], 3 * nen, len(points)
    shape = {0: (M, 3, 3), 1: (M, nen, 3), 2: (M, 6, nd), 3: (M, nd, nd), 4: (nq, M, nd, nd), 5: (M, nd, nd), 6: (M, nd, nd)}[what]
    out = _out_buffer(out, shape, dev, dtype)
    flat = [v for row in points for v in row]
    with torch.cuda.device(dev):
        check(lib.femb_solid(kind, what, _p(x), _fp(x), _p(conn), _fp(conn), M, _host_doubles(flat), nq, float(E), float(nu), _p(out),
                             _stream(dev)), "femb_solid")
    return out


def solid_stress(kind, coords, elements, displacement, points, E, nu, single=True, device="cuda:0", dtype=torch.float32):
    dev = cuda_device(device)
    x, conn, u = real(coords, dev, dtype), index(elements, dev), real(displacement, dev, dtype)
    nen = _NEN[kind]
    if conn.shape[1] != nen:
        conn = conn[:, :nen].contiguous()
    if u.shape != x.shape:
        raise ValueError(f"displacement must be [N,3] like coords, got {tuple(u.shape)} vs {tuple(x.shape)}")
    M, nq = conn.shape[0], len(points)
    lead = (M,) if single else (nq, M)
    S = torch.empty(lead + (3, 3), device=dev, dtype=dtype)
    V = torch.empty(lead, device=dev, dtype=dtype)
    flat = [v for row in points for v in row]
    with torch.cuda.device(dev):
        check(lib.femb_solid_stress(kind, _p(x), _fp(x), _p(conn), _fp(conn), M, _p(u), _host_doubles(flat), nq, float(E), float(nu),
                                    1 if single else 0, _p(S), _p(V), _stream(dev)), "femb_solid_stress")
    return S, V


def stress_helper(what, t):
    t = torch.as_tensor(t)
    dev = cuda_device(t.device)
    t = real(t, dev, t.dtype)
    M = t.shape[0]
    out = torch.empty((M, 3, 3) if what == 0 else (M,), device=dev, dtype=t.dtype)
    with torch.cuda.device(dev):
        check(lib.femb_stress_helper(what, _p(t), _fp(t), M, _p(out), _stream(dev)), "femb_stress_helper")
    return out


def shell(kind, what, coords, elements, points=None, D=None, device="cuda:0", dtype=torch.float32):
    dev = cuda_device(device)
    x, conn = real(coords, dev, dtype), index(elements, dev)
    nen = _NEN[kind]
    M, nd = conn.shape[0], 6 * nen
    points = points if points is not None else [[0.0, 0.0, 0.0, 1.0]]
    nq = len(points)
    shape = {0: (M, 3, 3), 1: (M, 2, 2), 2: (M, nen, 2), 3: (M, 6, nd), 4: (M, nd, nd), 5: (M, nd, nd, nq)}[what]
    out = torch.empty(shape, device=dev, dtype=dtype)
    flat = [v for row in points for v in row]
    Dh = _host_doubles([float(v) for v in D.reshape(-1).tolist()]) if D is not None else None
    with torch.cuda.device(dev):
        check(lib.femb_shell(kind, what, _p(x), _fp(x), _p(conn), _fp(conn), M, _host_doubles(flat), nq, Dh, _p(out), _stream(dev)),
              "femb_shell")
    return out


def shell_ex(kind, what, coords, elements, factors=None, D=None, disp=None, device="cuda:0", dtype=torch.float32):
    dev = cuda_device(device)
    x, conn = real(coords, dev, dtype), index(elements, dev)
    nen = _NEN[kind]
    M, nd = conn.shape[0], 6 * nen
    factors = factors if factors is not None else [[1.0, 1.0, 1.0, 1.0, 1.0]]
    nq = len(factors)
    shape = {0: (M, 3, 3), 1: (M, 2, 2), 2: (M, nen, 2), 3: (M, 6, nd), 4: (M, nd, nd), 5: (M, nd, nd, nq), 7: (M, 6, nd),
             8: (M, 6, nd, nq), 9: (M, 6)}[what]
    out = torch.empty(shape, device=dev, dtype=dtype)
    u = real(disp, dev, dtype) if disp is not None else None
    if what == 9 and (u is None or u.dim() != 2 or u.shape[1] != 6 or u.shape[0] != x.shape[0]):
        raise ValueError("shell stress needs the displacement as [N,6] (one row per node of coords)")
    flat = [v for row in factors for v in row]
    Dh = _host_doubles([float(v) for v in D.reshape(-1).tolist()]) if D is not None else None
    with torch.cuda.device(dev):
        check(lib.femb_shell_ex(kind, what, _p(x), _fp(x), _p(conn), _fp(conn), M, _host_doubles(flat), nq, Dh, _p(u), _p(out), _stream(dev)),
              "femb_shell_ex")
    return out


def shell_normal(coords, elements, device="cuda:0"):
    dev = cuda_device(device)
    x = torch.as_tensor(coords)
    x = real(x, dev, x.dtype if x.dtype in (torch.float32, torch.float64) else torch.float32)
    conn = index(elements, dev)
    out = torch.empty((conn.shape[0], 3), device=dev, dtype=x.dtype)
    with torch.cuda.device(dev):
        check(lib.femb_shell_normal(_p(x), _fp(x), _p(conn), _fp(conn), conn.shape[0], conn.shape[1], _p(out), _stream(dev)), "femb_shell_normal")
    return out


def shell_rotate_K(K, unit):
    dev = K.device
    K = real(K, dev, torch.float64)
    R = real(unit, dev, torch.float64)
    M, nd, _ = K.shape
    if tuple(R.shape) != (M, 3, 3):
        raise ValueError(f"unit must be [M,3,3], got {tuple(R.shape)}")
    out = torch.empty_like(K)
    with torch.cuda.device(dev):
        check(lib.femb_shell_rotate_operator(_p(K), _p(R), 8, M, nd, _p(out), _stream(dev)), "femb_shell_rotate_operator")
    return out


def shell_local_coordinates(coords, elements, unit, device="cuda:0", dtype=torch.float32):
    dev = cuda_device(device)
    x, conn = real(coords, dev, dtype), index(elements, dev)
    R = real(unit, dev, dtype)
    M, nen = conn.shape
    if tuple(R.shape) != (M, 3, 3):
        raise ValueError(f"unit must be [M,3,3], got {tuple(R.shape)}")
    out = torch.empty((M, nen, 3), device=dev, dtype=dtype)
    with torch.cuda.device(dev):
        check(lib.femb_shell_local_coordinates(_p(x), _fp(x), _p(conn), _fp(conn), M, nen, _p(R), _p(out), _stream(dev)),
              "femb_shell_local_coordinates")
    return out


def shell_local_displacement(elements, displacement, unit, device="cuda:0"):
    dev = cuda_device(device)
    conn = index(elements, dev)
    u = torch.as_tensor(displacement)
    u = real(u, dev, u.dtype if u.dtype in (torch.float32, torch.float64) else torch.float32)
    R = real(unit, dev, u.dtype)
    M, nen = conn.shape
    if u.dim() != 2 or u.shape[1] != 6 or tuple(R.shape) != (M, 3, 3):
        raise ValueError(f"expected displacement [N,6] and unit [M,3,3], got {tuple(u.shape)} and {tuple(R.shape)}")
    out = torch.empty((M, nen, 6), device=dev, dtype=u.dtype)
    with torch.cuda.device(dev):
        check(lib.femb_shell_local_displacement(_p(conn), _fp(conn), M, nen, _p(u), _p(R), _fp(u), _p(out), _stream(dev)),
              "femb_shell_local_displacement")
    return out


def shell_postprocess(NMQ, t, z, device="cuda:0", dtype=torch.float32):
    dev = cuda_device(device)
    v = real(NMQ, dev, dtype)
    if v.dim() != 2 or v.shape[1] < 6:
        raise ValueError(f"NMQ must be [M,6] or [M,8], got {tuple(v.shape)}")
    M = v.shape[0]
    out = torch.empty((8, M), device=dev, dtype=dtype)
    with torch.cuda.device(dev):
        check(lib.femb_shell_postprocess(_p(v), _fp(v), M, v.shape[1], float(t), float(z), _p(out), _stream(dev)), "femb_shell_postprocess")
    return out


def face_forces(normals, stress, device="cuda:0"):
    dev = cuda_device(device)
    s = torch.as_tensor(stress)
    dt = s.dtype if s.dtype in (torch.float32, torch.float64) else torch.float32
    s, n = real(s, dev, dt), real(normals, dev, dt)
    M, nf = n.shape[0], n.shape[1]
    if tuple(s.shape) != (M, 3, 3) or n.shape[2] != 3:
        raise ValueError(f"expected normals [M,nf,3] and stress [M,3,3], got {tuple(n.shape)} and {tuple(s.shape)}")
    out = torch.empty((M, nf, 3), device=dev, dtype=dt)
    with torch.cuda.device(dev):
        check(lib.femb_face_forces(_p(n), _p(s), _fp(s), M, nf, _p(out), _stream(dev)), "femb_face_forces")
    return out


def shared_face_forces_sum(pairs, forces, device="cuda:0"):
    dev = cuda_device(device)
    pr = torch.as_tensor(pairs).to(device=dev, dtype=torch.int64).contiguous()
    f = torch.as_tensor(forces)
    f = real(f, dev, f.dtype if f.dtype in (torch.float32, torch.float64) else torch.float32)
    S = pr.shape[0]
    if tuple(pr.shape[1:]) != (2, 2) or f.dim() != 3 or f.shape[2] != 3:
        raise ValueError(f"expected pairs [S,2,2] and forces [M,nf,3], got {tuple(pr.shape)} and {tuple(f.shape)}")
    if S and (int(pr[:, :, 0].max()) >= f.shape[0] or int(pr[:, :, 1].max()) >= f.shape[1] or int(pr.min()) < 0):
        raise IndexError("shared-face pair refers to an element / local face outside element_forces")
    out = torch.empty((S, 3), device=dev, dtype=f.dtype)
    with torch.cuda.device(dev):
        check(lib.femb_shared_face_forces_sum(_p(pr), S, _p(f), _fp(f), f.shape[1], _p(out), _stream(dev)), "femb_shared_face_forces_sum")
    return out


def wedge_face_normals(coords, elements, device="cuda:0", dtype=torch.float32):
    dev = cuda_device(device)
    x, conn = real(coords, dev, dtype), index(elements, dev)
    out = torch.empty((conn.shape[0], 5, 3), device=dev, dtype=dtype)
    with torch.cuda.device(dev):
        check(lib.femb_wedge_face_normals(_p(x), _fp(x), _p(conn), _fp(conn), conn.shape[0], conn.shape[1], _p(out), _stream(dev)),
              "femb_wedge_face_normals")
    return out


def shell_extrude(coords, tri, quad, thickness, eps=1e-8, device="cuda:0", dtype=torch.float32):
    dev = cuda_device(device)
    x = real(coords, dev, dtype)
    N = x.shape[0]
    conns, plans, outs = [], [], []
    for c, nen in ((tri, 3), (quad, 4)):
        c = index(c if c is not None else torch.empty((0, nen), dtype=torch.int64), dev).reshape(-1, nen)
        if c.numel() and (int(c.max()) >= N or int(c.min()) < 0):
            raise IndexError("shell connectivity refers to a node outside coords")
        conns.append(c)
        plans.append(cached_plan(c, N, dev) if c.shape[0] else None)
        outs.append(torch.empty((c.shape[0], 2 * nen), device=dev, dtype=c.dtype))
    x3 = torch.empty((2 * N, 3), device=dev, dtype=dtype)
    with torch.cuda.device(dev):
        st = _stream(dev)
        check(lib.femb_shell_extrude(plans[0].handle if plans[0] else None, plans[1].handle if plans[1] else None, _p(x), _fp(x), N,
                                     float(thickness), float(eps), _p(x3), st), "femb_shell_extrude")
        for c, o, nen in zip(conns, outs, (3, 4)):
            check(lib.femb_extrude_connectivity(_p(c), _fp(c), c.shape[0], nen, N, _p(o), st), "femb_extrude_connectivity")
    return x3, outs[0], outs[1]


def vtk_read(file_path):
    import numpy as np
    h, npnt, ncell, csize, isf = C.c_void_p(), C.c_int64(), C.c_int64(), C.c_int64(), C.c_int32()
    check(lib.femb_vtk_open(str(file_path).encode(), C.byref(h), C.byref(npnt), C.byref(ncell), C.byref(csize), C.byref(isf)), "femb_vtk_open")
    try:
        pts = np.empty((npnt.value, 3), dtype=np.float64)
        cells = np.empty(csize.value, dtype=np.int64)
        types = np.empty(ncell.value, dtype=np.int32)
        check(lib.femb_vtk_read(h, pts.ctypes.data_as(C.c_void_p), cells.ctypes.data_as(C.c_void_p), None), "femb_vtk_read")
        if lib.femb_vtk_read(h, None, None, types.ctypes.data_as(C.c_void_p)) != 0:
            types = None
    finally:
        lib.femb_vtk_close(h)
    return pts, cells, types, bool(isf.value)


def to_c3d4(kind, elements, device="cuda:0"):
    dev = cuda_device(device)
    conn = index(elements, dev)
    k = {C3D10: 8, C3D8: 6, C3D6: 3, C3D20: 24}[kind]
    if conn.shape[1] != _NEN[kind]:
        conn = conn[:, :_NEN[kind]].contiguous()
    out = torch.empty((conn.shape[0] * k, 4), device=dev, dtype=torch.int64)
    with torch.cuda.device(dev):
        check(lib.femb_to_c3d4(kind, _p(conn), _fp(conn), conn.shape[0], _p(out), _stream(dev)), "femb_to_c3d4")
    return out



def entities(ent_kind, elements, device="cuda:0", want_surface=True, want_shared=True):
    dev = cuda_device(device)
    conn = index(elements, dev)
    M = conn.shape[0]
    nf, nfn = _ENT[ent_kind]
    plan, K, S = C.c_void_p(), C.c_int64(), C.c_int64()
    with torch.cuda.device(dev):
        st = _stream(dev)
        check(lib.femb_entities_create(ent_kind, _p(conn), _fp(conn), M, conn.shape[1], st, C.byref(plan), C.byref(K), C.byref(S)),
              "femb_entities_create")
        try:
            faces = extra = pairs = None
            if want_surface:
                faces = torch.empty((K.value, nfn), device=dev, dtype=torch.int64)
                extra = torch.empty((K.value,), device=dev, dtype=torch.int64)
                check(lib.femb_entities_surface(plan, _p(faces), _p(extra), st), "femb_entities_surface")
            if want_shared:
                pairs = torch.empty((S.value, 2, 2), device=dev, dtype=torch.int64)
                check(lib.femb_entities_shared(plan, _p(pairs), st), "femb_entities_shared")
            torch.cuda.current_stream(dev).synchronize()
        finally:
            lib.femb_entities_destroy(plan)
    return faces, extra, pairs


def surface_normals(coords, faces, extra, second, device="cuda:0", dtype=torch.float32):
    dev = cuda_device(device)
    x = real(coords, dev, dtype)
    out = torch.empty((faces.shape[0], 3), device=dev, dtype=dtype)
    with torch.cuda.device(dev):
        check(lib.femb_surface_normals(_p(x), _fp(x), _p(faces), _p(extra), faces.shape[0], faces.shape[1], second, _p(out), _stream(dev)),
              "femb_surface_normals")
    return out


def face_normals_area(kind, coords, elements, device="cuda:0", dtype=torch.float32):
    dev = cuda_device(device)
    x, conn = real(coords, dev, dtype), index(elements, dev)
    nf = 4 if kind == C3D4 else 6
    out = torch.empty((conn.shape[0], nf, 3), device=dev, dtype=dtype)
    with torch.cuda.device(dev):
        check(lib.femb_face_normals_area(kind, _p(x), _fp(x), _p(conn), _fp(conn), conn.shape[0], conn.shape[1], _p(out), _stream(dev)),
              "femb_face_normals_area")
    return out



class CsrPlan:

    def __init__(self, elements, n_nodes=None, device="cuda:0"):
        self.dev = cuda_device(device)
        conn = index(elements, self.dev)
        self.M, self.nen = conn.shape
        self.n_nodes = int(n_nodes) if n_nodes is not None else (int(conn.max().item()) + 1 if self.M else 1)
        h, nnz = C.c_void_p(), C.c_int64()
        with torch.cuda.device(self.dev):
            try:
                check(lib.femb_csr_plan_create(_p(conn), _fp(conn), self.M, self.nen, self.n_nodes, _stream(self.dev), C.byref(h), C.byref(nnz)),
                      "femb_csr_plan_create")
            except _lib.FembError as exc:
                if "outside [0, n_nodes)" in str(exc):
                    raise IndexError(f"connectivity holds a node index outside [0, {self.n_nodes})") from exc
                raise
        self.handle, self.nnz_nodes = h, nnz.value
        L = self.M * self.nen
        self.nbytes = L * (8 + self.nen) + 8 * (self.n_nodes + 1) + 4 * self.nnz_nodes + (20 * L if self.nen == 4 else 0)
        self._fin = weakref.finalize(self, lib.femb_csr_plan_destroy, h)
        self._patterns = {}

    def pattern(self, ndof):
        if ndof not in self._patterns:
            n = self.n_nodes * ndof
            crow = torch.empty(n + 1, device=self.dev, dtype=torch.int32)
            col = torch.empty(self.nnz_nodes * ndof * ndof, device=self.dev, dtype=torch.int32)
            with torch.cuda.device(self.dev):
                check(lib.femb_csr_plan_pattern(self.handle, ndof, _p(crow), _p(col), _stream(self.dev)), "femb_csr_plan_pattern")
            self._patterns[ndof] = (crow, col)
        return self._patterns[ndof]

    def assemble(self, Ke, ndof, out=None):
        Ke = real(Ke, self.dev, torch.float64)
        assert Ke.shape == (self.M, self.nen * ndof, self.nen * ndof), (Ke.shape, self.M, self.nen, ndof)
        vals = out if out is not None else torch.empty(self.nnz_nodes * ndof * ndof, device=self.dev, dtype=torch.float64)
        with torch.cuda.device(self.dev):
            check(lib.femb_csr_assemble(self.handle, ndof, _p(Ke), _p(vals), _stream(self.dev)), "femb_csr_assemble")
        return vals

    def assemble_c3d4(self, coords, kind, E=0.0, nu=0.0, out=None, check_singular=True):
        k = {"poisson": 0, "elasticity": 1}[kind]
        d2 = 1 if k == 0 else 9
        x = real(coords, self.dev, torch.float64)
        vals = out if out is not None else torch.empty(self.nnz_nodes * d2, device=self.dev, dtype=torch.float64)
        flag = torch.zeros(1, device=self.dev, dtype=torch.int32)
        with torch.cuda.device(self.dev):
            check(lib.femb_csr_assemble_c3d4(self.handle, k, _p(x), float(E), float(nu), _p(vals), _p(flag), _stream(self.dev)),
                  "femb_csr_assemble_c3d4")
        if check_singular and int(flag.item()):
            raise ValueError("Singular matrix encountered while computing B matrix.")
        return vals

    def ebe_apply(self, Ke, u, ndof, unit=None, dtype=torch.float64):
        Ke, u = real(Ke, self.dev, dtype), real(u, self.dev, dtype)
        un = real(unit, self.dev, dtype) if unit is not None else None
        y = torch.empty((self.n_nodes, ndof), device=self.dev, dtype=dtype)
        assert u.shape[0] == self.n_nodes, "displacement rows must equal the plan's node count"
        with torch.cuda.device(self.dev):
            check(lib.femb_ebe_apply(self.handle, ndof, _p(Ke), _p(u), _p(un), _fp(u), _p(y), _stream(self.dev)), "femb_ebe_apply")
        return y

    def ebe_diag(self, Ke, ndof, dtype=torch.float64, col0=False):
        Ke = real(Ke, self.dev, dtype)
        assert Ke.shape == (self.M, self.nen * ndof, self.nen * ndof), (Ke.shape, self.M, self.nen, ndof)
        out = torch.empty((self.n_nodes, ndof), device=self.dev, dtype=dtype)
        with torch.cuda.device(self.dev):
            check(lib.femb_ebe_diag(self.handle, ndof, _p(Ke), _fp(Ke), 1 if col0 else 0, _p(out), _stream(self.dev)), "femb_ebe_diag")
        return out

    def node_average(self, elem_values, dtype=None):
        v = torch.as_tensor(elem_values)
        v = real(v, self.dev, dtype if dtype is not None else (v.dtype if v.dtype in (torch.float32, torch.float64) else torch.float64))
        assert v.shape == (self.M,), (v.shape, self.M)
        out = torch.empty(self.n_nodes, device=self.dev, dtype=v.dtype)
        with torch.cuda.device(self.dev):
            check(lib.femb_node_average(self.handle, _p(v), _fp(v), _p(out), _stream(self.dev)), "femb_node_average")
        return out


def p1_to_p2(coords, elements, device, dtype):
    dev = cuda_device(device)
    x = torch.as_tensor(coords).to(dev)
    if x.dtype not in (torch.float32, torch.float64):
        x = x.to(torch.float64)
    x = x.contiguous()
    conn = index(elements, dev)
    M, N = conn.shape[0], x.shape[0]
    h, ne = C.c_void_p(), C.c_int64()
    with torch.cuda.device(dev):
        check(lib.femb_p2_create(_p(conn), _fp(conn), M, N, _stream(dev), C.byref(h), C.byref(ne)), "femb_p2_create")
        try:
            E = ne.value
            conn10 = torch.empty((M, 10), device=dev, dtype=torch.int32)
            xo = torch.empty((N + E, 3), device=dev, dtype=dtype)
            edges = torch.empty((E, 2), device=dev, dtype=torch.int32)
            check(lib.femb_p2_fill(h, _p(conn), _fp(conn), _p(x), _fp(x), xo.element_size(), _p(conn10), _p(xo), _p(edges), _stream(dev)),
                  "femb_p2_fill")
        finally:
            lib.femb_p2_destroy(h)
    return xo, conn10, edges


_PLAN_CACHE: "collections.OrderedDict" = collections.OrderedDict()
PLAN_CACHE_BYTES = int(float(os.environ.get("FEMB_PLAN_CACHE_GB", "16")) * 2 ** 30)


def cached_plan(elements, n_nodes, device) -> CsrPlan:
    if not torch.is_tensor(elements):
        return CsrPlan(torch.as_tensor(elements).clone(), n_nodes, device)
    e = elements
    key = (id(e), e.data_ptr(), tuple(e.shape), e.dtype, e._version, str(e.device), int(n_nodes), str(device))
    plan = _PLAN_CACHE.get(key)
    if plan is None:
        plan = CsrPlan(e, n_nodes, device)
        plan._keepalive = e
        _PLAN_CACHE[key] = plan
        while len(_PLAN_CACHE) > 1 and (len(_PLAN_CACHE) > 8 or sum(p.nbytes for p in _PLAN_CACHE.values()) > PLAN_CACHE_BYTES):
            _PLAN_CACHE.popitem(last=False)
    else:
        _PLAN_CACHE.move_to_end(key)
    return plan



def spmv(crow, col, val, x):
    dev = val.device
    n = crow.numel() - 1
    xx = x.reshape(-1).contiguous()
    y = torch.empty(n, device=dev, dtype=torch.float64)
    with torch.cuda.device(dev):
        check(lib.femb_spmv(n, val.numel(), _p(crow), _p(col), _p(val), _p(xx), _p(y), _stream(dev)), "femb_spmv")
    return y.reshape(x.shape) if x.numel() == n else y


def jacobi(crow, col, val, mask=None):
    dev = val.device
    n = crow.numel() - 1
    out = torch.empty(n, device=dev, dtype=torch.float64)
    with torch.cuda.device(dev):
        check(lib.femb_csr_jacobi(n, _p(crow), _p(col), _p(val), _p(mask), _p(out), _stream(dev)), "femb_csr_jacobi")
    return out


STATUS = {0: "converged", 1: "breakdown", 2: "maxiter"}


def cg_solve(crow, col, val, F, mask=None, minv=None, u_init=None, tol=1e-10, max_iter=1000, eps=1e-30, check_every=16):
    dev = val.device
    n = crow.numel() - 1
    Ff = F.to(device=dev, dtype=torch.float64).reshape(-1).contiguous()
    assert Ff.numel() == n, (Ff.numel(), n)
    u = torch.zeros(n, device=dev, dtype=torch.float64) if u_init is None else \
        u_init.to(device=dev, dtype=torch.float64).reshape(-1).clone().contiguous()
    work = torch.empty(4 * n, device=dev, dtype=torch.float64)
    res = CGResult()
    with torch.cuda.device(dev):
        check(lib.femb_cg_solve(n, val.numel(), _p(crow), _p(col), _p(val), _p(Ff), _p(mask), _p(minv), _p(u), _p(work), float(tol),
                                int(max_iter), float(eps), int(check_every), C.byref(res), _stream(dev)), "femb_cg_solve")
    info = {"iterations": res.iterations, "status": STATUS.get(res.status, "?"), "rs": res.rs, "loop_ms": res.loop_ms,
            "index_bytes": res.index_bytes}
    return u.reshape(F.shape), info


def cg_solve_multi(mats, F, mask=None, minv=None, u_init=None, tol=1e-10, max_iter=1000, eps=1e-30, check_every=16):
    dev = mats[0][2].device
    n = mats[0][0].numel() - 1
    Ff = F.to(device=dev, dtype=torch.float64).reshape(-1).contiguous()
    assert Ff.numel() == n and all(m[0].numel() - 1 == n for m in mats)
    u = torch.zeros(n, device=dev, dtype=torch.float64) if u_init is None else \
        u_init.to(device=dev, dtype=torch.float64).reshape(-1).clone().contiguous()
    work = torch.empty(4 * n, device=dev, dtype=torch.float64)
    k = len(mats)
    nnz = (C.c_int64 * k)(*[m[2].numel() for m in mats])
    crow = (C.c_void_p * k)(*[m[0].data_ptr() for m in mats])
    col = (C.c_void_p * k)(*[m[1].data_ptr() for m in mats])
    val = (C.c_void_p * k)(*[m[2].data_ptr() for m in mats])
    res = CGResult()
    with torch.cuda.device(dev):
        check(lib.femb_cg_solve_multi(n, k, nnz, crow, col, val, _p(Ff), _p(mask), _p(minv), _p(u), _p(work), float(tol), int(max_iter),
                                      float(eps), int(check_every), C.byref(res), _stream(dev)), "femb_cg_solve_multi")
    info = {"iterations": res.iterations, "status": STATUS.get(res.status, "?"), "rs": res.rs, "loop_ms": res.loop_ms}
    return u.reshape(F.shape), info


def cg_solve_operator(apply, R, tol=1e-8, max_iter=1000, check_every=8, device="cuda:0"):
    dev = cuda_device(device)
    Rf = R.to(device=dev, dtype=torch.float64).reshape(-1).contiguous()
    n = Rf.numel()
    u = torch.zeros(n, device=dev, dtype=torch.float64)
    work = torch.empty(3 * n, device=dev, dtype=torch.float64)
    views = {u.data_ptr(): u, (work.data_ptr() + 8 * n): work[n:2 * n]}
    Ap = work[2 * n:]
    raised = []

    def _cb(_ctx, xptr, yptr, _stream_):
        try:
            x = views[int(xptr)]
            assert int(yptr) == Ap.data_ptr()
            y = apply(x.reshape(R.shape))
            Ap.copy_(torch.as_tensor(y).to(device=dev, dtype=torch.float64).reshape(-1))
            return 0
        except BaseException as exc:
            raised.append(exc)
            return 1

    cb = _lib.APPLY_FN(_cb)
    res = CGResult()
    with torch.cuda.device(dev):
        rc = lib.femb_cg_solve_operator(n, cb, None, _p(Rf), _p(u), _p(work), float(tol), int(max_iter), int(check_every), C.byref(res),
                                        _stream(dev))
    if raised:
        raise raised[0]
    check(rc, "femb_cg_solve_operator")
    info = {"iterations": res.iterations, "status": STATUS.get(res.status, "?"), "rs": res.rs, "loop_ms": res.loop_ms}
    return u.reshape(R.shape), info



class MultiVec:

    def __init__(self, data):
        assert data.dim() == 2 and data.dtype == torch.float64 and data.is_contiguous() and data.shape[0] <= 8
        self.data, self.k, self.n, self.dev = data, data.shape[0], data.shape[1], data.device

    @classmethod
    def from_columns(cls, X, dev):
        return cls(torch.as_tensor(X).to(device=dev, dtype=torch.float64).t().contiguous())

    def columns(self):
        return self.data.t().contiguous()

    def cols(self, a, b):
        return MultiVec(self.data[a:b])

    def gram(self, other, w=None):
        G = (C.c_double * (self.k * other.k))()
        with torch.cuda.device(self.dev):
            check(lib.femb_mv_gram(self.n, self.k, _p(self.data), self.n, other.k, _p(other.data), other.n, _p(w), G, _stream(self.dev)),
                  "femb_mv_gram")
        return torch.tensor(list(G), dtype=torch.float64).reshape(self.k, other.k)

    def update_into(self, coef, out, beta=0.0):
        coef = torch.as_tensor(coef, dtype=torch.float64).reshape(self.k, out.k)
        Ch = _host_doubles(coef.reshape(-1).tolist())
        with torch.cuda.device(self.dev):
            check(lib.femb_mv_update(self.n, self.k, _p(self.data), self.n, out.k, Ch, float(beta), _p(out.data), out.n, _stream(self.dev)),
                  "femb_mv_update")
        return out

    def scale_mask(self, scale=None, mask=None):
        with torch.cuda.device(self.dev):
            check(lib.femb_mv_scale_mask(self.n, self.k, _p(self.data), self.n, _p(scale), _p(mask), _stream(self.dev)), "femb_mv_scale_mask")
        return self



class Bsr3:

    def __init__(self, brow, bcol, bval):
        self.brow, self.bcol, self.bval = brow, bcol, bval
        self.nb, self.nnzb, self.dev = brow.numel() - 1, bcol.numel(), bval.device

    @classmethod
    def from_csr_values(cls, brow, bcol, csr_val):
        assert csr_val.numel() == 9 * bcol.numel(), (csr_val.numel(), bcol.numel())
        bval = torch.empty((bcol.numel(), 3, 3), device=csr_val.device, dtype=torch.float64)
        with torch.cuda.device(csr_val.device):
            check(lib.femb_csr_bsr3_convert(1, brow.numel() - 1, _p(brow), _p(csr_val), _p(bval), _stream(csr_val.device)),
                  "femb_csr_bsr3_convert")
        return cls(brow, bcol, bval)

    def to_csr_values(self):
        out = torch.empty(9 * self.nnzb, device=self.dev, dtype=torch.float64)
        with torch.cuda.device(self.dev):
            check(lib.femb_csr_bsr3_convert(0, self.nb, _p(self.brow), _p(self.bval), _p(out), _stream(self.dev)), "femb_csr_bsr3_convert")
        return out

    def spmv(self, x):
        xx = x.to(device=self.dev, dtype=torch.float64).reshape(-1).contiguous()
        assert xx.numel() == 3 * self.nb
        y = torch.empty(3 * self.nb, device=self.dev, dtype=torch.float64)
        with torch.cuda.device(self.dev):
            check(lib.femb_spmv_bsr3(self.nb, self.nnzb, _p(self.brow), _p(self.bcol), _p(self.bval), _p(xx), _p(y), _stream(self.dev)),
                  "femb_spmv_bsr3")
        return y.reshape(x.shape)

    def jacobi(self, mask=None):
        out = torch.empty(3 * self.nb, device=self.dev, dtype=torch.float64)
        with torch.cuda.device(self.dev):
            check(lib.femb_bsr3_jacobi(self.nb, _p(self.brow), _p(self.bcol), _p(self.bval), _p(mask), _p(out), _stream(self.dev)),
                  "femb_bsr3_jacobi")
        return out

    def cg_solve(self, F, mask=None, minv=None, u_init=None, tol=1e-10, max_iter=1000, eps=1e-30, check_every=16):
        n = 3 * self.nb
        Ff = F.to(device=self.dev, dtype=torch.float64).reshape(-1).contiguous()
        assert Ff.numel() == n, (Ff.numel(), n)
        u = torch.zeros(n, device=self.dev, dtype=torch.float64) if u_init is None else \
            u_init.to(device=self.dev, dtype=torch.float64).reshape(-1).clone().contiguous()
        work = torch.empty(4 * n, device=self.dev, dtype=torch.float64)
        res = CGResult()
        with torch.cuda.device(self.dev):
            check(lib.femb_cg_solve_bsr3(self.nb, self.nnzb, _p(self.brow), _p(self.bcol), _p(self.bval), _p(Ff), _p(mask), _p(minv), _p(u),
                                         _p(work), float(tol), int(max_iter), float(eps), int(check_every), C.byref(res),
                                         _stream(self.dev)), "femb_cg_solve_bsr3")
        info = {"iterations": res.iterations, "status": STATUS.get(res.status, "?"), "rs": res.rs, "loop_ms": res.loop_ms}
        return u.reshape(F.shape), info
```

include/femb200.h:

```cpp
#ifndef FEMB200_H
#define FEMB200_H

#include <stdint.h>

#ifdef __cplusplus
extern "C" {
#endif

typedef void* femb_stream;

enum {
  FEMB_OK = 0,
  FEMB_ERR_ARG = 1,
  FEMB_ERR_CUDA = 2,
  FEMB_ERR_SINGULAR = 3,
  FEMB_ERR_NCCL = 4,
  FEMB_ERR_UNSUPPORTED = 5
};

const char* femb_last_error(void);
int femb_version(void);


enum { FEMB_C3D4 = 4, FEMB_C3D6 = 6, FEMB_C3D8 = 8, FEMB_C3D10 = 10, FEMB_C3D15 = 15, FEMB_C3D20 = 20, FEMB_S3 = 103, FEMB_S4 = 104 };

int femb_elem_volumes(int kind, const void* coords, int fp, const void* conn, int ib, int64_t M, int conn_stride,
                      void* vol, femb_stream stream);

int femb_c3d4(int what, const void* coords, int fp, const void* conn, int ib, int64_t M, double E, double nu, void* out,
              int32_t* flag, femb_stream stream);

int femb_solid(int kind, int what, const void* coords, int fp, const void* conn, int ib, int64_t M, const double* pts_host,
               int nq, double E, double nu, void* out, femb_stream stream);

int femb_default_points(int kind, double* pts_host);

int femb_mass_points(int kind, double* pts_host);

int femb_shape_tables(int kind, const double* pts_host, int nq, double* N_host, double* dN_host);

int femb_solid_stress(int kind, const void* coords, int fp, const void* conn, int ib, int64_t M, const void* disp,
                      const double* pts_host, int nq, double E, double nu, int single, void* stress, void* vm,
                      femb_stream stream);

int femb_shell(int kind, int what, const void* coords, int fp, const void* conn, int ib, int64_t M, const double* pts_host,
               int nq, const double* D6_host, void* out, femb_stream stream);

int femb_shell_ex(int kind, int what, const void* coords, int fp, const void* conn, int ib, int64_t M, const double* fac_host,
                  int nq, const double* D6_host, const void* disp, void* out, femb_stream stream);

int femb_shell_local_coordinates(const void* coords, int fp, const void* conn, int ib, int64_t M, int nen, const void* unit, void* out,
                                 femb_stream stream);

int femb_shell_normal(const void* coords, int fp, const void* conn, int ib, int64_t M, int nen, void* out, femb_stream stream);
int femb_shell_rotate_operator(const void* K, const void* unit, int fp, int64_t M, int nd, void* out, femb_stream stream);

int femb_shell_local_displacement(const void* conn, int ib, int64_t M, int nen, const void* disp, const void* unit, int fp,
                                  void* out, femb_stream stream);

int femb_shell_postprocess(const void* nmq, int fp, int64_t M, int ncol, double t, double z, void* out, femb_stream stream);

int femb_face_forces(const void* normals, const void* stress, int fp, int64_t M, int nf, void* out, femb_stream stream);
int femb_shared_face_forces_sum(const int64_t* pairs, int64_t S, const void* forces, int fp, int nf, void* out, femb_stream stream);

int femb_stress_helper(int what, const void* in, int fp, int64_t M, void* out, femb_stream stream);

int femb_to_c3d4(int kind, const void* conn, int ib, int64_t M, int64_t* out, femb_stream stream);

typedef struct femb_p2_plan femb_p2_plan;
int femb_p2_create(const void* conn, int ib, int64_t M, int64_t n_nodes, femb_stream stream, femb_p2_plan** plan, int64_t* n_edges);
int femb_p2_fill(femb_p2_plan* plan, const void* conn, int ib, const void* coords, int fp_in, int fp_out, int32_t* conn10,
                 void* coords_out, int32_t* edges, femb_stream stream);
int femb_p2_destroy(femb_p2_plan* plan);

enum {
  FEMB_ENT_TET_FACES = 0,
  FEMB_ENT_HEX_FACES = 1,
  FEMB_ENT_WEDGE_QUADS = 2,
  FEMB_ENT_WEDGE_TRIS = 3,
  FEMB_ENT_TRI_EDGES = 4,
  FEMB_ENT_QUAD_EDGES = 5
};
typedef struct femb_entity_plan femb_entity_plan;
int femb_entities_create(int ent_kind, const void* conn, int ib, int64_t M, int conn_stride, femb_stream stream,
                         femb_entity_plan** plan, int64_t* n_surface, int64_t* n_shared);
int femb_entities_surface(femb_entity_plan* plan, int64_t* faces, int64_t* extra, femb_stream stream);
int femb_entities_shared(femb_entity_plan* plan, int64_t* pairs, femb_stream stream);
int femb_entities_destroy(femb_entity_plan* plan);

int femb_surface_normals(const void* coords, int fp, const int64_t* faces, const int64_t* extra, int64_t K, int nfn,
                         int second, void* normals, femb_stream stream);
int femb_face_normals_area(int kind, const void* coords, int fp, const void* conn, int ib, int64_t M, int conn_stride,
                           void* out, femb_stream stream);

int femb_wedge_face_normals(const void* coords, int fp, const void* conn, int ib, int64_t M, int conn_stride, void* out,
                            femb_stream stream);

typedef struct femb_csr_plan femb_csr_plan;
int femb_csr_plan_create(const void* conn, int ib, int64_t M, int nen, int64_t n_nodes, femb_stream stream,
                         femb_csr_plan** plan, int64_t* nnz_nodes);
int femb_csr_plan_pattern(femb_csr_plan* plan, int ndof, int32_t* crow, int32_t* col, femb_stream stream);
int femb_csr_assemble(femb_csr_plan* plan, int ndof, const double* Ke, double* vals, femb_stream stream);
int femb_csr_assemble_c3d4(femb_csr_plan* plan, int kind, const double* coords, double E, double nu, double* vals,
                           int32_t* flag, femb_stream stream);
int femb_csr_plan_destroy(femb_csr_plan* plan);

int femb_spmv(int64_t n_rows, int64_t nnz, const int32_t* crow, const int32_t* col, const double* val, const double* x, double* y,
              femb_stream stream);

int femb_ebe_apply(femb_csr_plan* plan, int ndof, const void* Ke, const void* u, const void* unit, int fp, void* y,
                   femb_stream stream);

int femb_shell_extrude(femb_csr_plan* tri, femb_csr_plan* quad, const void* coords, int fp, int64_t N, double thickness, double eps,
                       void* coords3d, femb_stream stream);
int femb_extrude_connectivity(const void* conn, int ib, int64_t M, int nen, int64_t N, void* out, femb_stream stream);

int femb_ebe_diag(femb_csr_plan* plan, int ndof, const void* Ke, int fp, int col0, void* out, femb_stream stream);

int femb_node_average(femb_csr_plan* plan, const void* elem_values, int fp, void* out, femb_stream stream);

int femb_csr_bsr3_convert(int to_bsr, int64_t nb, const int32_t* brow, const double* in, double* out, femb_stream stream);
int femb_spmv_bsr3(int64_t nb, int64_t nnzb, const int32_t* brow, const int32_t* bcol, const double* bval, const double* x, double* y,
                   femb_stream stream);
int femb_bsr3_jacobi(int64_t nb, const int32_t* brow, const int32_t* bcol, const double* bval, const uint8_t* mask, double* minv,
                     femb_stream stream);

typedef struct femb_cg_result {
  int32_t iterations;
  int32_t status;
  double rs;
  double loop_ms;
  int32_t index_bytes;
} femb_cg_result;

int femb_cg_solve(int64_t n, int64_t nnz, const int32_t* crow, const int32_t* col, const double* val, const double* F,
                  const uint8_t* mask, const double* minv, double* u, double* work, double tol, int max_iter, double eps,
                  int check_every, femb_cg_result* result_host, femb_stream stream);

int femb_cg_solve_bsr3(int64_t nb, int64_t nnzb, const int32_t* brow, const int32_t* bcol, const double* bval, const double* F,
                       const uint8_t* mask, const double* minv, double* u, double* work, double tol, int max_iter, double eps,
                       int check_every, femb_cg_result* result_host, femb_stream stream);

int femb_cg_solve_multi(int64_t n, int nmat, const int64_t* nnz_host, const int32_t* const* crow_host,
                        const int32_t* const* col_host, const double* const* val_host, const double* F, const uint8_t* mask,
                        const double* minv, double* u, double* work, double tol, int max_iter, double eps, int check_every,
                        femb_cg_result* result_host, femb_stream stream);

typedef int (*femb_apply_fn)(void* ctx, const double* x, double* y, femb_stream stream);
int femb_cg_solve_operator(int64_t n, femb_apply_fn apply, void* ctx, const double* R, double* u, double* work, double tol,
                           int max_iter, int check_every, femb_cg_result* result_host, femb_stream stream);

int femb_mv_gram(int64_t n, int ki, const double* X, int64_t ldx, int kj, const double* Y, int64_t ldy, const double* w, double* G_host,
                 femb_stream stream);
int femb_mv_update(int64_t n, int ki, const double* X, int64_t ldx, int kj, const double* C_host, double beta, double* Y, int64_t ldy,
                   femb_stream stream);
int femb_mv_scale_mask(int64_t n, int k, double* X, int64_t ldx, const double* scale, const uint8_t* mask, femb_stream stream);

int femb_spmm_bsr3(int64_t nb, int64_t nnzb, const int32_t* brow, const int32_t* bcol, const double* kval, const double* mval,
                   const uint8_t* mask, int m, const double* X, int64_t ldx, double* YK, double* YM, int64_t ldy, femb_stream stream);
int femb_mb_gram(int64_t n, int ka, const double* A, int64_t lda, int kb, const double* B, int64_t ldb, double* G, femb_stream stream);
int femb_mb_combine(int64_t n, int k, const double* X, int64_t ldx, int mc, const double* C_host, double beta, double* Y, int64_t ldy,
                    femb_stream stream);
int femb_lobpcg_residual(int64_t n, int m, const double* X, int64_t ldx, const double* KX, const double* MX, int64_t ldk,
                         const double* lam_host, const double* dinv, int na, const int32_t* active, double* W, int64_t ldw,
                         double* norms, femb_stream stream);

int femb_csr_jacobi(int64_t n, const int32_t* crow, const int32_t* col, const double* val, const uint8_t* mask,
                    double* minv, femb_stream stream);

int femb_graph_from_pairs(const int64_t* pairs, int64_t S, int pair_stride, int64_t M, int32_t* crow, int32_t* col,
                          femb_stream stream);
int femb_graph_bfs(const int32_t* crow, const int32_t* col, int64_t M, const int64_t* sources, int n_sources, int32_t* dist,
                   int32_t* label, int32_t* levels_host, femb_stream stream);

int femb_subdomain_forces(const void* F, int fp, int64_t N, int n_sub, const void* free_vars, int64_t ntgt, const int64_t* tgt,
                          const int32_t* plus, const int32_t* minus, void* out, femb_stream stream);

typedef struct femb_vtk_mesh femb_vtk_mesh;
int femb_vtk_open(const char* path, femb_vtk_mesh** mesh, int64_t* n_points, int64_t* n_cells, int64_t* cells_size,
                  int32_t* points_are_float);
int femb_vtk_read(femb_vtk_mesh* mesh, double* points_host, int64_t* cells_host, int32_t* types_host);
int femb_vtk_close(femb_vtk_mesh* mesh);

int femb_dist_header_bytes(void);
int femb_dist_alloc(int64_t bytes, void** ptr, void* ipc_handle64);
int femb_dist_open(const void* ipc_handle64, void** ptr);
int femb_dist_close(void* ptr);
int femb_dist_free(void* ptr);
int femb_dist_reset(void* own_sym, femb_stream stream);

int femb_dist_cg_solve(int rank, int nranks, int64_t n_owned, int64_t n_interior, int64_t nnz, const int32_t* crow,
                       const int32_t* col, const double* val, const double* F, const uint8_t* mask, const double* minv,
                       double* u, double* work,
                       void* const* sym_host, int nnbr, const int32_t* nbr_host, const int32_t* send_ptr_host,
                       const int32_t* send_idx, const int64_t* ghost_off_host,
                       const int32_t* bptr, const uint8_t* bk, const int32_t* boff, double tol, int max_iter, double eps,
                       int check_every, int block, femb_cg_result* result_host, femb_stream stream);

#ifdef __cplusplus
}
#endif
#endif
```

Baseline: 2227.

## Fuse CG vector update into SpMV kernel with per-tile dataflow counters

Adds a single cooperative CG kernel that performs the u/r/p update for the previous iteration tile by tile inside the SpMV loop. Fine-grained release/acquire counters let a block proceed once the tiles its rows reference (column reach precomputed per tile) have been updated, replacing the separate vector-update kernel and its grid-wide barrier. The payoff is one kernel launch per iteration instead of two, plus less re-reading of p and Ap. The cost is spin-waiting, a setup pass to compute reach, and the requirement that all blocks be co-resident. It stays gated on bandwidth and occupancy checks.

New measurement: 1442, median of 6. -35.2%, worse.

```diff
diff --git a/cuda-powered-mesh-handling-and-iterative-solvers_b200/csrc/krylov.cu b/cuda-powered-mesh-handling-and-iterative-solvers_b200/csrc/krylov.cu
--- a/cuda-powered-mesh-handling-and-iterative-solvers_b200/csrc/krylov.cu
+++ b/cuda-powered-mesh-handling-and-iterative-solvers_b200/csrc/krylov.cu
@@ -44,6 +44,21 @@
   cg_k1_epilogue_n<SPMV_THREADS>(dot, partial, st, eps, guards);
 }
 
+__device__ __forceinline__ void cg_merged_alpha_beta(CGState* __restrict__ st, double a, double b, double c, double eps, int guards) {
+  st->pAp = a;
+  const double rs = st->rs_old, alpha = rs / (a + eps);
+  if (guards && (fabs(a) < eps || a < 0.0 || !isfinite(alpha))) {
+    st->stop = 1, st->status = 1, st->iterations = st->it + 1;
+  } else {
+    double rs_new = rs - 2.0 * alpha * b + alpha * alpha * c;
+    if (!(rs_new > 0.0)) rs_new = 0.0;
+    const double beta = rs_new / (rs + eps);
+    st->alpha = alpha, st->beta = beta, st->rs_new = rs_new;
+    st->fin = 0;
+    if (guards && !isfinite(beta)) st->fin = 1, st->fin_status = 1;
+  }
+}
+
 template <int THREADS>
 __device__ __forceinline__ void cg_k1_epilogue3_n(double dot, double e0, double e1, double* __restrict__ partial, CGState* __restrict__ st,
                                                   double eps, int guards, double tol) {
@@ -64,18 +79,7 @@
     a = block_sum<THREADS>(a), b = block_sum<THREADS>(b), c = block_sum<THREADS>(c);
     if (threadIdx.x == 0) {
       st->ticket1 = 0;
-      st->pAp = a;
-      const double rs = st->rs_old, alpha = rs / (a + eps);
-      if (guards && (fabs(a) < eps || a < 0.0 || !isfinite(alpha))) {
-        st->stop = 1, st->status = 1, st->iterations = st->it + 1;
-      } else {
-        double rs_new = rs - 2.0 * alpha * b + alpha * alpha * c;
-        if (!(rs_new > 0.0)) rs_new = 0.0;
-        const double beta = rs_new / (rs + eps);
-        st->alpha = alpha, st->beta = beta, st->rs_new = rs_new;
-        st->fin = 0;
-        if (guards && !isfinite(beta)) st->fin = 1, st->fin_status = 1;
-      }
+      cg_merged_alpha_beta(st, a, b, c, eps, guards);
     }
   }
 }
@@ -181,23 +185,41 @@
 
 __global__ void __launch_bounds__(TMA_THREADS) idx16_encode_kernel(long long n, const int* __restrict__ crow, const int* __restrict__ col,
                                                                    unsigned short* __restrict__ col16, unsigned char* __restrict__ tile_ok,
-                                                                   int* __restrict__ bad) {
+                                                                   int* __restrict__ bad, int* __restrict__ reach, int* __restrict__ fwd) {
+  __shared__ int wmax[TMA_THREADS / 32];
   const long long ntiles = (n + TMA_THREADS - 1) / TMA_THREADS;
   for (long long t = blockIdx.x; t < ntiles; t += gridDim.x) {
     const long long r = t * TMA_THREADS + threadIdx.x;
     bool ok = true;
+    int mx = -1;
     if (r < n) {
       const int a = __ldg(crow + r), b = __ldg(crow + r + 1);
       long long prev = r;
       for (int j = a; j < b; ++j) {
-        const long long c = __ldg(col + j), d = j == a ? prev - c : c - prev;
-        ok = ok && d >= (j == a ? 0 : 1) && d <= 65535;
-        col16[j] = (unsigned short)d;
-        prev = c;
+        const int cj = __ldg(col + j);
+        mx = max(mx, cj);
+        if (col16) {
+          const long long c = cj, d = j == a ? prev - c : c - prev;
+          ok = ok && d >= (j == a ? 0 : 1) && d <= 65535;
+          col16[j] = (unsigned short)d;
+          prev = c;
+        }
       }
     }
     ok = __syncthreads_and(ok);
-    if (threadIdx.x == 0) {
+    if (reach) {
+      mx = __reduce_max_sync(0xffffffffu, mx);
+      if ((threadIdx.x & 31) == 0) wmax[threadIdx.x >> 5] = mx;
+      __syncthreads();
+      if (threadIdx.x == 0) {
+        for (int w = 1; w < TMA_THREADS / 32; ++w) mx = max(mx, wmax[w]);
+        const int rt = mx < 0 ? -1 : mx / TMA_THREADS;
+        reach[t] = rt;
+        if (rt > t) atomicMax(fwd, (int)(rt - t));
+      }
+      __syncthreads();
+    }
+    if (threadIdx.x == 0 && col16) {
       tile_ok[t] = ok ? 1 : 0;
       if (!ok) atomicAdd(bad, 1);
     }
@@ -368,6 +390,19 @@
   }
 }
 
+__device__ __forceinline__ void cg_merged_finish(CGState* __restrict__ st, double a, bool move_p, int max_iter, double tol) {
+  st->rs_new = a;
+  if (sqrt(a) < tol) {
+    st->stop = 1, st->status = 0, st->iterations = st->it + 1;
+  } else if (!move_p) {
+    st->stop = 1, st->status = st->fin_status, st->iterations = st->it + 1;
+  } else {
+    st->rs_old = a;
+    st->it += 1;
+    if (st->it >= max_iter) st->stop = 2, st->status = 2, st->iterations = max_iter;
+  }
+}
+
 __global__ void __launch_bounds__(VEC_THREADS) cg_merged_kernel(long long n, double* __restrict__ u, double* __restrict__ r, double* __restrict__ p,
                                                                 const double* __restrict__ Ap, const double* __restrict__ minv,
                                                                 double* __restrict__ partial, CGState* __restrict__ st, int max_iter, double tol) {
@@ -400,16 +435,143 @@
     a = block_sum<VEC_THREADS>(a);
     if (threadIdx.x == 0) {
       st->ticket2 = 0;
-      st->rs_new = a;
-      if (sqrt(a) < tol) {
-        st->stop = 1, st->status = 0, st->iterations = st->it + 1;
-      } else if (!move_p) {
-        st->stop = 1, st->status = st->fin_status, st->iterations = st->it + 1;
+      cg_merged_finish(st, a, move_p, max_iter, tol);
+    }
+  }
+}
+
+__device__ __forceinline__ unsigned ld_acquire_gpu(const unsigned* p) {
+  unsigned v;
+  asm volatile("ld.acquire.gpu.global.u32 %0, [%1];" : "=r"(v) : "l"(p) : "memory");
+  return v;
+}
+
+struct FusedUpdate {
+  long long n, ntiles;
+  double *u, *r, *p;
+  const double *Ap, *minv;
+  double alpha, beta;
+  bool move_p;
+  unsigned* cnt;
+  const int* reach;
+  int lead;
+  unsigned epoch;
+  double rz = 0.0;
+  long long have = -1;
+  long long row = 0;
+  double pi = 0.0, ri = 0.0, ai = 0.0, ui = 0.0, mi = 0.0;
+  long long pend = -1;
+  long long ready = -1;
+  long long mine = -1;
+  int need = -1;
+
+  __device__ __forceinline__ long long tile(long long k) const { return blockIdx.x + k * gridDim.x; }
+  __device__ __forceinline__ void load(long long k) {
+    have = tile(k) < ntiles ? k : -1;
+    row = tile(k) * TMA_THREADS + threadIdx.x;
+    if (have >= 0 && row < n) {
+      pi = p[row], ri = r[row], ai = Ap[row], ui = u[row];
+      if (minv) mi = minv[row];
+    }
+  }
+  __device__ __forceinline__ void apply() {
+    if (have >= 0 && row < n) {
+      const double rn = ri - alpha * ai, zn = minv ? mi * rn : rn;
+      u[row] = ui + alpha * pi;
+      r[row] = rn;
+      rz += rn * zn;
+      if (move_p) p[row] = zn + beta * pi;
+    }
+    pend = have;
+  }
+  __device__ __forceinline__ void release() {
+    if (threadIdx.x == 0 && pend >= 0) {
+      __threadfence();
+      asm volatile("red.release.gpu.global.add.u32 [%0], 1;" ::"l"(cnt + pend) : "memory");
+      mine = pend;
+    }
+    pend = -1;
+  }
+  __device__ __forceinline__ void begin() {
+    for (int j = 0; j < lead; ++j) load(j), apply();
+    __syncthreads();
+    if (threadIdx.x == 0) {
+      __threadfence();
+      for (int j = 0; j < lead && tile(j) < ntiles; ++j) {
+        asm volatile("red.release.gpu.global.add.u32 [%0], 1;" ::"l"(cnt + j) : "memory");
+        mine = j;
+      }
+    }
+    pend = -1;
+  }
+  __device__ __forceinline__ void top(long long k) {
+    release();
+    if (threadIdx.x == 0) need = __ldg(reach + tile(k));
+    load(k + lead);
+  }
+  __device__ __forceinline__ void wait(long long) {
+    if (threadIdx.x == 0 && need >= 0 && need / gridDim.x > ready) {
+      const long long w = need / gridDim.x;
+      auto done = [&](long long v) {
+        return (int)(ld_acquire_gpu(cnt + v) - epoch * (unsigned)min((long long)gridDim.x, ntiles - v * gridDim.x)) >= 0;
+      };
+      if (mine > w && done(mine)) {
+        ready = mine;
       } else {
-        st->rs_old = a;
-        st->it += 1;
-        if (st->it >= max_iter) st->stop = 2, st->status = 2, st->iterations = max_iter;
-      }
+        while (!done(w)) {
+        }
+        ready = w;
+      }
+    }
+  }
+  __device__ __forceinline__ void bottom() { apply(); }
+  __device__ __forceinline__ void end() { release(); }
+};
+
+template <bool IDX16>
+__global__ void __launch_bounds__(TMA_THREADS) cg_fused_kernel(long long n, long long nnz, const int* crow, const int* col,
+                                                               const unsigned short* col16, const unsigned char* tile_ok, const double* val,
+                                                               double* u, double* r, double* p, double* Ap, const unsigned char* mask,
+                                                               const double* minv, double* partial, CGState* st, double eps, int guards,
+                                                               double tol, int max_iter, long long pin, unsigned* cnt, const int* reach,
+                                                               int lead) {
+  if (st->stop) return;
+  const bool move_p = st->fin == 0;
+  const int it = st->it;
+  const bool spmv = move_p && it + 1 < max_iter;
+  const long long ntiles = (n + TMA_THREADS - 1) / TMA_THREADS;
+  FusedUpdate U{n, ntiles, u, r, p, Ap, minv, st->alpha, st->beta, move_p, cnt, reach, lead, (unsigned)it + 1u};
+  double dot = 0.0, extra[2] = {0.0, 0.0};
+  if (spmv) {
+    if constexpr (IDX16)
+      dot = spmv_tma16_rows<TMA16_STAGES, TMA16_CAP, false, FusedUpdate>(n, nnz, crow, col, col16, tile_ok, val, p, Ap, mask, false, true, r,
+                                                                         extra, nullptr, pin, minv, &U);
+    else
+      dot = spmv_tma_rows<1, false, TMA_THREADS, TMA_STAGES, TMA_CAP, NoHaloWait, NoDep, FusedUpdate>(
+          n, nnz, crow, col, val, p, Ap, mask, false, true, 0x7fffffffffffffffll, NoHaloWait(), r, extra, NoDep(), nullptr, pin, minv, &U);
+  } else {
+    for (long long k = 0; U.tile(k) < ntiles; ++k) U.load(k), U.apply();
+  }
+  const double t0 = block_sum<TMA_THREADS>(dot), t1 = block_sum<TMA_THREADS>(extra[0]), t2 = block_sum<TMA_THREADS>(extra[1]),
+               t3 = block_sum<TMA_THREADS>(U.rz);
+  const int G = gridDim.x;
+  __shared__ bool last;
+  if (threadIdx.x == 0) {
+    partial[blockIdx.x] = t0, partial[G + blockIdx.x] = t1, partial[2 * G + blockIdx.x] = t2, partial[3 * G + blockIdx.x] = t3;
+    __threadfence();
+    last = atomicAdd(&st->ticket1, 1u) == G - 1;
+  }
+  __syncthreads();
+  if (last) {
+    __threadfence();
+    const volatile double* vp = partial;
+    double a = 0.0, b = 0.0, c = 0.0, d = 0.0;
+    for (int k = threadIdx.x; k < G; k += TMA_THREADS) a += vp[k], b += vp[G + k], c += vp[2 * G + k], d += vp[3 * G + k];
+    a = block_sum<TMA_THREADS>(a), b = block_sum<TMA_THREADS>(b), c = block_sum<TMA_THREADS>(c), d = block_sum<TMA_THREADS>(d);
+    if (threadIdx.x == 0) {
+      st->ticket1 = 0;
+      cg_merged_finish(st, d, move_p, max_iter, tol);
+      if (!st->stop) cg_merged_alpha_beta(st, a, b, c, eps, guards);
     }
   }
 }
@@ -548,6 +710,17 @@
 #undef FEMB_BSR
 #undef FEMB_BSRV
 #undef FEMB_SPMV_ARGS
+}
+
+template <typename... KArgs, typename... Args>
+static cudaError_t launch_coop(void (*kern)(KArgs...), int grid, int block, size_t smem, cudaStream_t s, Args... args) {
+  cudaLaunchConfig_t cfg = {};
+  cfg.gridDim = dim3((unsigned)grid), cfg.blockDim = dim3((unsigned)block), cfg.dynamicSmemBytes = smem, cfg.stream = s;
+  cudaLaunchAttribute at[1];
+  at[0].id = cudaLaunchAttributeCooperative;
+  at[0].val.cooperative = 1;
+  cfg.attrs = at, cfg.numAttrs = 1;
+  return cudaLaunchKernelEx(&cfg, kern, static_cast<KArgs>(args)...);
 }
 
 static int spmv_grid(long long n, int lanes, bool merged = false) {
@@ -629,7 +802,7 @@
   static const bool idx32_env = getenv("FEMB_SPMV_IDX32") != nullptr;
   bool use16 = !idx32_env && merged && nmat == 1 && lanes[0] == 101 && max_iter >= 16;
   const long long ntiles16 = (n + TMA_THREADS - 1) / TMA_THREADS;
-  const size_t flags_off = 256, col16_off = flags_off + (((size_t)ntiles16 + 255) & ~(size_t)255);
+  const size_t flags_off = 0, col16_off = flags_off + (((size_t)ntiles16 + 255) & ~(size_t)255);
   if (use16) {
     const size_t need16 = col16_off + 2 * (((size_t)mats[0].nnz + 7) & ~(size_t)7);
     if (ctx->idx16_bytes < need16) {
@@ -641,20 +814,8 @@
       else ctx->idx16 = nullptr, use16 = false, cudaGetLastError();
     }
   }
-  if (use16) {
-    unsigned char* base16 = static_cast<unsigned char*>(ctx->idx16);
-    static_assert(2 * sizeof(CGState) + sizeof(int) <= 512 && 512 + sizeof(int) <= SOLVE_PINNED_BYTES, "pinned status buffer");
-    int* bad_host = reinterpret_cast<int*>(static_cast<unsigned char*>(ctx->pinned) + 512);
-    FEMB_CUDA(cudaMemsetAsync(base16, 0, sizeof(int), s));
-    idx16_encode_kernel<<<(int)std::min<long long>(ntiles16, (long long)SMS * 16), TMA_THREADS, 0, s>>>(
-        n, mats[0].crow, mats[0].col, reinterpret_cast<unsigned short*>(base16 + col16_off), base16 + flags_off, reinterpret_cast<int*>(base16));
-    FEMB_LAUNCH_CHECK();
-    FEMB_CUDA(cudaMemcpyAsync(bad_host, base16, sizeof(int), cudaMemcpyDeviceToHost, s));
-    FEMB_CUDA(cudaStreamSynchronize(s));
-    use16 = (long long)*bad_host * 100 <= ntiles16;
-  }
-  const unsigned short* col16 = use16 ? reinterpret_cast<const unsigned short*>(static_cast<unsigned char*>(ctx->idx16) + col16_off) : nullptr;
-  const unsigned char* tile_ok = use16 ? static_cast<unsigned char*>(ctx->idx16) + flags_off : nullptr;
+  static const bool two_kernel_env = getenv("FEMB_CG_TWO_KERNEL") != nullptr;
+  bool fused = !two_kernel_env && merged && nmat == 1 && lanes[0] == 101;
   for (int m = 0; m < nmat; ++m) {
     g1[m] = spmv_grid(n, lanes[m], merged && m == nmat - 1);
     if (use16) g1[m] = tma16_grid(n);
@@ -663,7 +824,8 @@
   const int g2 = grid_for(n, VEC_THREADS, 8);
   static const int vec_waves = getenv("FEMB_VEC_WAVES") ? atoi(getenv("FEMB_VEC_WAVES")) : 8;
   const int g2v = grid_for(n, VEC_THREADS, vec_waves);
-  const size_t need = 256 + sizeof(double) * (size_t)std::max(3 * gmax, g2);
+  const size_t slots = (size_t)std::max(4 * gmax, g2), region_off = 256 + sizeof(double) * slots;
+  const size_t need = region_off + 8 * (size_t)ntiles16 + 2 * sizeof(int);
   if (ctx->dev_scratch_bytes < need) {
     if (ctx->graph_exec) cudaGraphExecDestroy(ctx->graph_exec), ctx->graph_exec = nullptr, ctx->graph_key_bytes = 0;
     FEMB_CUDA(cudaStreamSynchronize(s));
@@ -675,6 +837,46 @@
   static_assert(sizeof(CGState) <= 256, "state slot");
   CGState* st = static_cast<CGState*>(ctx->dev_scratch);
   double* partial = reinterpret_cast<double*>(static_cast<unsigned char*>(ctx->dev_scratch) + 256);
+  unsigned* wave_cnt = reinterpret_cast<unsigned*>(static_cast<unsigned char*>(ctx->dev_scratch) + region_off);
+  int* reach = reinterpret_cast<int*>(wave_cnt + ntiles16);
+  int* pass = reach + ntiles16;
+  int lead = 0;
+  if (use16 || fused) {
+    unsigned char* base16 = static_cast<unsigned char*>(ctx->idx16);
+    static_assert(2 * sizeof(CGState) <= 512 && 512 + 2 * sizeof(int) <= SOLVE_PINNED_BYTES, "pinned status buffer");
+    int* pass_host = reinterpret_cast<int*>(static_cast<unsigned char*>(ctx->pinned) + 512);
+    FEMB_CUDA(cudaMemsetAsync(pass, 0, 2 * sizeof(int), s));
+    idx16_encode_kernel<<<(int)std::min<long long>(ntiles16, (long long)SMS * 16), TMA_THREADS, 0, s>>>(
+        n, mats[0].crow, mats[0].col, use16 ? reinterpret_cast<unsigned short*>(base16 + col16_off) : nullptr, use16 ? base16 + flags_off : nullptr,
+        pass, fused ? reach : nullptr, pass + 1);
+    FEMB_LAUNCH_CHECK();
+    FEMB_CUDA(cudaMemcpyAsync(pass_host, pass, 2 * sizeof(int), cudaMemcpyDeviceToHost, s));
+    FEMB_CUDA(cudaStreamSynchronize(s));
+    if (use16) use16 = (long long)pass_host[0] * 100 <= ntiles16;
+    if (use16) g1[0] = tma16_grid(n);
+    else g1[0] = spmv_grid(n, lanes[0], merged);
+    if (fused) {
+      const long long fwd = pass_host[1], g32 = tma_grid(n, 1);
+      fused = (fwd + g32 - 1) / g32 + 1 <= 8;
+      static const int slack = getenv("FEMB_CG_FUSED_SLACK") ? atoi(getenv("FEMB_CG_FUSED_SLACK")) : 1;
+      lead = (int)((fwd + g1[0] - 1) / g1[0] + 1 + slack);
+    }
+  }
+  if (fused) {
+    const size_t smem = use16 ? TMA16_SMEM : TMA_SMEM;
+    int per_sm = 0;
+    if (use16) {
+      cudaFuncSetAttribute(cg_fused_kernel<true>, cudaFuncAttributeMaxDynamicSharedMemorySize, (int)smem);
+      cudaOccupancyMaxActiveBlocksPerMultiprocessor(&per_sm, cg_fused_kernel<true>, TMA_THREADS, smem);
+    } else {
+      cudaFuncSetAttribute(cg_fused_kernel<false>, cudaFuncAttributeMaxDynamicSharedMemorySize, (int)smem);
+      cudaOccupancyMaxActiveBlocksPerMultiprocessor(&per_sm, cg_fused_kernel<false>, TMA_THREADS, smem);
+    }
+    fused = (long long)per_sm * num_sms() >= g1[0];
+  }
+  const unsigned short* col16 = use16 ? reinterpret_cast<const unsigned short*>(static_cast<unsigned char*>(ctx->idx16) + col16_off) : nullptr;
+  const unsigned char* tile_ok = use16 ? static_cast<unsigned char*>(ctx->idx16) + flags_off : nullptr;
+  if (fused) FEMB_CUDA(cudaMemsetAsync(wave_cnt, 0, sizeof(unsigned) * (size_t)((ntiles16 + g1[0] - 1) / g1[0]), s));
   if (mask) cg_mask_kernel<<<g2, VEC_THREADS, 0, s>>>(n, u, mask);
   col16_hint = col16, tile_ok_hint = tile_ok;
   for (int m = 0; m < nmat; ++m)
@@ -693,12 +895,14 @@
     double tol, eps;
     long long pin;
     const void* col16;
+    int fused, lead;
   } key;
   memset(&key, 0, sizeof(key));
   static_assert(sizeof(GraphKey) <= sizeof(ctx->graph_key), "graph key buffer");
   key.n = n, key.nmat = nmat, key.check_every = check_every, key.max_iter = max_iter, key.guards = guards, key.merged = merged ? 1 : 0;
   key.pdl = pdl_mode(), key.g2 = g2, key.g2v = g2v, key.mask = mask, key.minv = minv, key.u = u, key.work = work, key.st = st, key.partial = partial;
   key.tol = tol, key.eps = eps, key.pin = spmv_pin_entries(mats[nmat - 1].nnz), key.col16 = col16;
+  key.fused = fused ? 1 : 0, key.lead = lead;
   for (int m = 0; m < nmat; ++m) {
     key.lanes[m] = lanes[m], key.g1[m] = g1[m];
     key.nnz[m] = mats[m].nnz, key.crow[m] = mats[m].crow, key.col[m] = mats[m].col, key.val[m] = mats[m].val, key.block[m] = mats[m].block;
@@ -709,12 +913,23 @@
   if (!no_cache && ctx->graph_exec && ctx->graph_key_bytes == sizeof(key) && memcmp(ctx->graph_key, &key, sizeof(key)) == 0) exec = ctx->graph_exec;
   if (!exec) {
   FEMB_CUDA(cudaStreamBeginCapture(s, cudaStreamCaptureModeThreadLocal));
+#define FEMB_FUSED_ARGS n, mats[0].nnz, mats[0].crow, mats[0].col, col16, tile_ok, mats[0].val, u, r, p, Ap, mask, minv, partial, st, eps, \
+                        guards, tol, max_iter, key.pin, wave_cnt, (const int*)reach, lead
   for (int k = 0; k < check_every; ++k) {
     for (int m = 0; m + 1 < nmat; ++m)
       nnz_hint = mats[m].nnz, launch_spmv<false>(lanes[m], g1[m], s, n, mats[m].crow, mats[m].col, mats[m].val, p, Ap, nullptr, nullptr, st, 0.0, m ? 2 : 0);
     const int last = nmat - 1;
     nnz_hint = mats[last].nnz;
-    if (merged) {
+    if (fused) {
+      const cudaError_t le = use16 ? launch_coop(cg_fused_kernel<true>, g1[0], TMA_THREADS, TMA16_SMEM, s, FEMB_FUSED_ARGS)
+                                   : launch_coop(cg_fused_kernel<false>, g1[0], TMA_THREADS, TMA_SMEM, s, FEMB_FUSED_ARGS);
+      if (le != cudaSuccess) {
+        cudaStreamEndCapture(s, &graph);
+        if (graph) cudaGraphDestroy(graph);
+        set_error(std::string("fused CG kernel launch: ") + cudaGetErrorString(le));
+        return FEMB_ERR_CUDA;
+      }
+    } else if (merged) {
       const bool pdl = pdl_enabled() && nmat == 1 && lanes[last] >= 100 && lanes[last] < 200;
       pdl_hint = pdl && k > 0 && (pdl_mode() & 2);
       pin_hint = pdl ? spmv_pin_entries(mats[last].nnz) : 0;
@@ -730,6 +945,7 @@
       cg_direction_kernel<<<g2, VEC_THREADS, 0, s>>>(n, r, p, minv, st);
     }
   }
+#undef FEMB_FUSED_ARGS
   cudaError_t ce = cudaStreamEndCapture(s, &graph);
   if (ce != cudaSuccess) {
     set_error(std::string("cudaStreamEndCapture: ") + cudaGetErrorString(ce));
@@ -751,7 +967,13 @@
   hst[0].stop = hst[1].stop = 0;
   bool stopped = false;
   cudaEventRecord(tev[0], s);
-  for (int l = 0; l < launches && !stopped; ++l) {
+  if (fused) {
+    nnz_hint = mats[0].nnz, pin_hint = key.pin, col16_hint = col16, tile_ok_hint = tile_ok;
+    launch_spmv<true>(lanes[0], g1[0], s, n, mats[0].crow, mats[0].col, mats[0].val, p, Ap, mask, partial, st, eps, guards, r, tol, minv);
+    pin_hint = 0, col16_hint = nullptr, tile_ok_hint = nullptr;
+    if (cudaGetLastError() != cudaSuccess) rc = FEMB_ERR_CUDA, set_error("fused CG: first SpMV launch failed");
+  }
+  for (int l = 0; l < launches && !stopped && rc == FEMB_OK; ++l) {
     if (cudaGraphLaunch(exec, s) != cudaSuccess || cudaMemcpyAsync(&hst[l & 1], st, sizeof(CGState), cudaMemcpyDeviceToHost, s) != cudaSuccess ||
         cudaEventRecord(ev[l & 1], s) != cudaSuccess) {
       set_error(std::string("CG graph launch: ") + cudaGetErrorString(cudaGetLastError()));
@@ -783,6 +1005,7 @@
   result_host->rs = fin->rs_new;
   result_host->loop_ms = ms;
   result_host->index_bytes = use16 ? 2 : 4;
+  result_host->fused = fused ? 1 : 0;
   return FEMB_OK;
 }
 
@@ -919,5 +1142,6 @@
   result_host->rs = h.rs_new;
   result_host->loop_ms = ms;
   result_host->index_bytes = 0;
+  result_host->fused = 0;
   return FEMB_OK;
 }
diff --git a/cuda-powered-mesh-handling-and-iterative-solvers_b200/csrc/spmv_dev.cuh b/cuda-powered-mesh-handling-and-iterative-solvers_b200/csrc/spmv_dev.cuh
--- a/cuda-powered-mesh-handling-and-iterative-solvers_b200/csrc/spmv_dev.cuh
+++ b/cuda-powered-mesh-handling-and-iterative-solvers_b200/csrc/spmv_dev.cuh
@@ -162,6 +162,13 @@
 struct NoDep {
   __device__ __forceinline__ void operator()() const {}
 };
+struct NoStep {
+  __device__ __forceinline__ void begin() {}
+  __device__ __forceinline__ void top(long long) {}
+  __device__ __forceinline__ void wait(long long) {}
+  __device__ __forceinline__ void bottom() {}
+  __device__ __forceinline__ void end() {}
+};
 
 template <typename... KArgs, typename... Args>
 inline cudaError_t launch_pdl(void (*kern)(KArgs...), int grid, int block, size_t smem, cudaStream_t s, bool pdl, Args... args) {
@@ -183,13 +190,14 @@
 constexpr size_t TMA_SMEM = (size_t)TMA_STAGES * TMA_CAP * 12;
 
 template <int LR, bool NC, int THREADS = TMA_THREADS, int STAGES = TMA_STAGES, int CAP = TMA_CAP, typename Wait = NoHaloWait,
-          typename Dep = NoDep>
+          typename Dep = NoDep, typename Step = NoStep>
 __device__ __forceinline__ double spmv_tma_rows(long long n, long long nnz, const int* __restrict__ crow, const int* __restrict__ col,
                                                 const double* __restrict__ val, const double* __restrict__ x, double* __restrict__ y,
                                                 const unsigned char* __restrict__ mask, bool accumulate, bool fused,
                                                 long long halo_row = 0x7fffffffffffffffll, Wait wait = Wait(),
                                                 const double* __restrict__ rvec = nullptr, double* extra = nullptr, Dep dep = Dep(),
-                                                const int* stop = nullptr, long long pin = 0, const double* __restrict__ wvec = nullptr) {
+                                                const int* stop = nullptr, long long pin = 0, const double* __restrict__ wvec = nullptr,
+                                                Step* step = nullptr) {
   constexpr int R = THREADS / LR;
   extern __shared__ __align__(128) unsigned char tma_smem[];
   double* vbuf = reinterpret_cast<double*>(tma_smem);
@@ -252,6 +260,7 @@
       return 0.0;
     }
   }
+  if (step) step->begin();
   for (long long k = 0;; ++k) {
     const long long t = blockIdx.x + k * gridDim.x;
     if (t >= ntiles) break;
@@ -264,6 +273,7 @@
       stage_tile(k + STAGES - 1, na, nb);
       bounds(k + STAGES, na, nb);
     }
+    if (step) step->top(k);
     const long long r = t * R + lr;
     int ra = 0, rb = 0;
     double x_own = 0.0, y_prev = 0.0, r_own = 0.0, w_own = 1.0;
@@ -280,6 +290,7 @@
         if (accumulate) y_prev = y[r];
       }
     }
+    if (step) step->wait(t);
     __syncthreads();
     const int a0 = base[s];
     double sum = 0.0;
@@ -318,8 +329,10 @@
       }
       y[r] = sum;
     }
-    __syncthreads();
-  }
+    if (step) step->bottom();
+    __syncthreads();
+  }
+  if (step) step->end();
   return dot;
 }
 
@@ -350,13 +363,13 @@
   return (int)std::max<long long>(1, std::min<long long>(tiles, (long long)SMS * TMA16_CTAS_PER_SM));
 }
 
-template <int STAGES, int CAP>
+template <int STAGES, int CAP, bool NC = true, typename Step = NoStep>
 __device__ __forceinline__ double spmv_tma16_rows(long long n, long long nnz, const int* __restrict__ crow, const int* __restrict__ col,
                                                   const unsigned short* __restrict__ col16, const unsigned char* __restrict__ tile_ok,
                                                   const double* __restrict__ val, const double* __restrict__ x, double* __restrict__ y,
                                                   const unsigned char* __restrict__ mask, bool accumulate, bool fused,
                                                   const double* __restrict__ rvec, double* extra, const int* stop, long long pin,
-                                                  const double* __restrict__ wvec) {
+                                                  const double* __restrict__ wvec, Step* step = nullptr) {
   static_assert(CAP % 8 == 0, "16-byte aligned stages");
   constexpr int R = TMA_THREADS;
   extern __shared__ __align__(128) unsigned char tma_smem[];
@@ -419,6 +432,7 @@
       return 0.0;
     }
   }
+  if (step) step->begin();
   for (long long k = 0;; ++k) {
     const long long t = blockIdx.x + k * gridDim.x;
     if (t >= ntiles) break;
@@ -427,6 +441,7 @@
       stage_tile(k + STAGES - 1, na, nb, nok);
       bounds(k + STAGES, na, nb, nok);
     }
+    if (step) step->top(k);
     const long long r = t * R + tid;
     int ra = 0, rb = 0;
     double x_own = 0.0, y_prev = 0.0, r_own = 0.0, w_own = 1.0;
@@ -434,13 +449,14 @@
     if (r < n) {
       ra = __ldg(crow + r), rb = __ldg(crow + r + 1);
       if (fused) {
-        x_own = __ldg(x + r);
+        x_own = ld_x<NC>(x + r);
         if (mask) keep = mask[r] != 0;
         if (rvec) r_own = rvec[r];
         if (wvec) w_own = wvec[r];
       }
       if (accumulate) y_prev = y[r];
     }
+    if (step) step->wait(t);
     __syncthreads();
     const int a0 = base[s];
     double sum = 0.0;
@@ -454,7 +470,7 @@
       for (; j + 7 < rb; j += 8) {
         double xv[8];
 #pragma unroll
-        for (int q = 0; q < 8; ++q) c += ds[j + q], xv[q] = __ldg(x + c);
+        for (int q = 0; q < 8; ++q) c += ds[j + q], xv[q] = ld_x<NC>(x + c);
 #pragma unroll
         for (int q = 0; q < 8; ++q) sum += vs[j + q] * xv[q];
       }
@@ -463,14 +479,14 @@
 #pragma unroll
         for (int q = 0; q < 7; ++q) {
           if (j + q < rb) c += ds[j + q];
-          xv[q] = (j + q < rb) ? __ldg(x + c) : 0.0;
+          xv[q] = (j + q < rb) ? ld_x<NC>(x + c) : 0.0;
         }
 #pragma unroll
         for (int q = 0; q < 7; ++q)
           if (j + q < rb) sum += vs[j + q] * xv[q];
       }
     } else {
-      for (int j = ra; j < rb; ++j) sum += ld_stream(val + j) * __ldg(x + ld_stream(col + j));
+      for (int j = ra; j < rb; ++j) sum += ld_stream(val + j) * ld_x<NC>(x + ld_stream(col + j));
     }
     if (r < n) {
       if (accumulate) sum += y_prev;
@@ -481,8 +497,10 @@
       }
       y[r] = sum;
     }
-    __syncthreads();
-  }
+    if (step) step->bottom();
+    __syncthreads();
+  }
+  if (step) step->end();
   return dot;
 }
 
diff --git a/cuda-powered-mesh-handling-and-iterative-solvers_b200/femb200/_lib.py b/cuda-powered-mesh-handling-and-iterative-solvers_b200/femb200/_lib.py
--- a/cuda-powered-mesh-handling-and-iterative-solvers_b200/femb200/_lib.py
+++ b/cuda-powered-mesh-handling-and-iterative-solvers_b200/femb200/_lib.py
@@ -11,7 +11,7 @@
 
 class CGResult(C.Structure):
     _fields_ = [("iterations", C.c_int32), ("status", C.c_int32), ("rs", C.c_double), ("loop_ms", C.c_double),
-                ("index_bytes", C.c_int32)]
+                ("index_bytes", C.c_int32), ("fused", C.c_int32)]
 
 
 APPLY_FN = C.CFUNCTYPE(C.c_int, c_vp, c_vp, c_vp, c_vp)
diff --git a/cuda-powered-mesh-handling-and-iterative-solvers_b200/femb200/ops.py b/cuda-powered-mesh-handling-and-iterative-solvers_b200/femb200/ops.py
--- a/cuda-powered-mesh-handling-and-iterative-solvers_b200/femb200/ops.py
+++ b/cuda-powered-mesh-handling-and-iterative-solvers_b200/femb200/ops.py
@@ -555,7 +555,7 @@
         check(lib.femb_cg_solve(n, val.numel(), _p(crow), _p(col), _p(val), _p(Ff), _p(mask), _p(minv), _p(u), _p(work), float(tol),
                                 int(max_iter), float(eps), int(check_every), C.byref(res), _stream(dev)), "femb_cg_solve")
     info = {"iterations": res.iterations, "status": STATUS.get(res.status, "?"), "rs": res.rs, "loop_ms": res.loop_ms,
-            "index_bytes": res.index_bytes}
+            "index_bytes": res.index_bytes, "fused": bool(res.fused)}
     return u.reshape(F.shape), info
 
 
diff --git a/include/femb200.h b/include/femb200.h
--- a/include/femb200.h
+++ b/include/femb200.h
@@ -131,6 +131,7 @@
   double rs;
   double loop_ms;
   int32_t index_bytes;
+  int32_t fused;
 } femb_cg_result;
 
 int femb_cg_solve(int64_t n, int64_t nnz, const int32_t* crow, const int32_t* col, const double* val, const double* F,
```
